# meffmadd/intro-tc-vae

Measured on AMD Instinct MI355X. Metric: images/sec (64x64x3, z=128, bs=64) intro-TC step, higher is better.
Workload: dtype f32 in/out/accumulate, conv products on split-fp16 MFMA (two scaled fp16 planes, 3 products, fp32-class); 1 GPU; c2: IntroTCSovler.train_step, conv arch, 64x64x3, z_dim=128, channels (64, 128, 256, 512), batch 64/GPU, Adam lr 2e-4, clip 100, N=10000; global_batch=64, parallelism=single, sync_bn=False

## Files before the change

### include/itcv_hip.h

```cpp
#ifndef ITCV_HIP_H
#define ITCV_HIP_H

#include <stddef.h>
#include <stdint.h>

#ifdef __cplusplus
extern "C" {
#endif

#define ITCV_ABI_VERSION 4

int itcv_abi_version(void);
const char* itcv_last_error(void);
int itcv_set_option(const char* name, int value);
int itcv_get_option(const char* name);

int itcv_profile_begin(void);
int itcv_profile_end(void);
int itcv_profile_get(int i, int* code, double* flop, float* ms);
int itcv_profile_clear(void);

size_t itcv_conv2d_packed_weight_elems(int Co, int Ci, int KS, int for_dgrad);
int itcv_conv2d_pack_weight(const float* w, float* wp, int Co, int Ci, int KS, int for_dgrad,
                            void* stream);
size_t itcv_conv2d_fwd_workspace(int B, int Ci, int H, int W, int Co, int KS);
int itcv_conv2d_fwd(const float* x, const float* wp, const float* bias, float* y, int B, int Ci,
                    int H, int W, int Co, int KS, int up2, void* ws, size_t ws_bytes, void* stream);
int itcv_conv2d_bf16s_supported(int Ci, int Co, int KS);
size_t itcv_conv2d_packed_weight_bytes_bf16s(int Co, int Ci, int KS, int for_dgrad, int ns);
int itcv_conv2d_pack_weight_bf16s(const float* w, void* wp, int Co, int Ci, int KS, int for_dgrad, int ns,
                                  void* stream);
size_t itcv_pack_desc_bytes(void);
int itcv_conv2d_pack_desc_bf16s(void* host_desc, const float* w, void* wp, int Co, int Ci, int KS, int for_dgrad,
                                int ns, int block0);
int itcv_conv2d_pack_weights_bf16s(const void* dev_table, int n, int total_blocks, int ns, void* stream);
size_t itcv_conv2d_fwd_bf16s_workspace(int B, int Ci, int H, int W, int Co, int KS);
int itcv_conv2d_fwd_bf16s(const float* x, const void* wp, const float* bias, float* y, int B, int Ci, int H,
                          int W, int Co, int KS, int up2, int ns, void* ws, size_t ws_bytes, void* stream);
#define ITCV_PLANES_F16X2 4
size_t itcv_planes_bytes(int B, int C, int HW, int ns);
int itcv_split_planes(const float* x, void* planes, int B, int C, int HW, int ns, void* stream);
int itcv_absmax(const float* x, size_t n, float* parts, void* stream);
int itcv_split_planes_scaled(const float* x, void* planes, int B, int C, int HW, int ns, const float* amax, void* stream);
size_t itcv_conv2d_fwd_bf16p_workspace(int B, int Ci, int H, int W, int Co, int KS, int ns);
int itcv_conv2d_fwd_bf16p(const void* xplanes, const void* wp, const float* bias, float* y, int B, int Ci, int H,
                          int W, int Co, int KS, int up2, int ns, void* ws, size_t ws_bytes, void* stream);
int itcv_conv2d_fwd_bf16p_stat_tiles(int B, int Ci, int H, int W, int Co, int KS, int ns);
int itcv_conv2d_fwd_bf16p_st(const void* xplanes, const void* wp, const float* bias, float* y, int B, int Ci, int H,
                             int W, int Co, int KS, int up2, int ns, float* tile_stats, void* ws, size_t ws_bytes,
                             void* stream);
int itcv_conv2d_wgrad_bf16p_supported(int B, int Ci, int H, int W, int Co, int KS);
size_t itcv_conv2d_wgrad_bf16p_workspace(int B, int Ci, int H, int W, int Co, int KS);
int itcv_conv2d_wgrad_bf16p(const void* xplanes, const void* dyplanes, float* dw, int B, int Ci, int H, int W,
                            int Co, int KS, int up2, int ns , int accumulate, void* ws, size_t ws_bytes,
                            void* stream);
int itcv_conv2d_wgrad_bf16p_slabs(int B, int Ci, int H, int W, int Co, int KS);
size_t itcv_wgrad_reduce_desc_bytes(void);
int itcv_wgrad_reduce_desc(void* host_desc, const float* const* slabs, const int* splits, int nsrc, float* dw, int Co,
                           int Ci, int accumulate, int block0);
int itcv_wgrad_reduce_many(const void* dev_table, int n, int total_blocks, void* stream);
int itcv_wgrad_reduce_max_descs(void);
size_t itcv_linear_workspace(int B, int K, int N);
int itcv_linear_fwd(const float* x, const float* w, const float* bias, float* y, int B, int K, int N, void* ws,
                    size_t ws_bytes, void* stream);
int itcv_linear_dgrad(const float* dy, const float* w, float* dx, int B, int K, int N, void* ws, size_t ws_bytes,
                      void* stream);
int itcv_linear_wgrad(const float* dy, const float* x, float* dw, int B, int K, int N, int accumulate, void* ws,
                      size_t ws_bytes, void* stream);
int itcv_conv2d_wgrad5_bf16p_supported(int Cs, int Cb, int H, int W);
size_t itcv_conv2d_wgrad5_bf16p_workspace(int B, int H);
int itcv_conv2d_wgrad5_bf16p(const float* small, const void* big_planes, float* dw, int B, int Cs, int H, int W,
                             int stem, int ns , const float* small_amax ,
                             int accumulate, void* ws, size_t ws_bytes, void* stream);
int itcv_conv2d_small_cout_supported(int Co, int KS);
int itcv_conv2d_small_cout_bf16p_supported(int C, int Co, int KS);
int itcv_conv2d_small_cout_fwd_bf16p(const void* xplanes, const float* w, const float* bias, float* y, int B, int C,
                                     int H, int W, int Co, int KS, int for_dgrad, int ns , void* stream);
int itcv_conv2d_small_cout_fwd(const float* x, const float* w, const float* bias, float* y, int B, int C,
                               int H, int W, int Co, int KS, int for_dgrad, void* stream);
int itcv_conv2d_small_cin_supported(int C, int KS);
int itcv_conv2d_small_cin_fwd(const float* x, const float* w, const float* bias, float* y, int B, int C, int H,
                              int W, int Co, int KS, int for_dgrad, void* stream);

int itcv_conv2d_small_cin_bf16x3_supported(int C, int Co, int KS, int W);
int itcv_conv2d_small_cin_fwd_bf16x3(const float* x, const float* w, const float* bias, float* y, int B, int C, int H,
                                     int W, int Co, int KS, int for_dgrad, int ns ,
                                     const float* x_amax , void* stream);
int itcv_conv2d_wgrad_bf16s_supported(int Ci, int H, int W, int Co, int KS);
int itcv_conv2d_wgrad_bf16s(const float* x, const float* dy, float* dw, int B, int Ci, int H, int W, int Co,
                            int KS, int ns, int accumulate, void* ws, size_t ws_bytes, void* stream);
size_t itcv_conv2d_wgrad_workspace(int B, int Ci, int H, int W, int Co, int KS);
int itcv_conv2d_wgrad(const float* x, const float* dy, float* dw, int B, int Ci, int H, int W,
                      int Co, int KS, int up2, int accumulate, void* ws, size_t ws_bytes, void* stream);
int itcv_conv2d_fwd_variant(int B, int Ci, int H, int W, int Co, int KS, int up2);
int itcv_conv2d_wgrad_variant(int B, int Ci, int H, int W, int Co, int KS, int up2);
size_t itcv_bias_grad_workspace(int B, int C, int HW);
int itcv_bias_grad(const float* dy, float* db, int B, int C, int HW, int accumulate, void* ws,
                   size_t ws_bytes, void* stream);

size_t itcv_bn_workspace(int B, int C, int HW);
int itcv_bn_moments(const float* x, double* sums, int B, int C, int HW, void* ws, size_t ws_bytes,
                    void* stream);
int itcv_bn_train_stats(const float* x, int B, int C, int HW, float eps, float momentum, float* running_mean,
                        float* running_var, int64_t* num_batches_tracked, float* mean, float* rstd, void* ws,
                        size_t ws_bytes, void* stream);
int itcv_bn_finalize(const double* sums, double count, float eps, float momentum, float* running_mean,
                     float* running_var, int64_t* num_batches_tracked, float* mean, float* rstd, int C,
                     void* stream);
int itcv_bn_finalize_uv(const double* sums, double count, float eps, float momentum, float* running_mean,
                        float* running_var, int64_t* num_batches_tracked, float* mean, float* rstd, float* unbiased_var,
                        int C, void* stream);
int itcv_bn_eval_stats(const float* running_mean, const float* running_var, float eps, float* mean,
                       float* rstd, int C, void* stream);
int itcv_bn_act_fwd(const float* x, const float* mean, const float* rstd, const float* gamma,
                    const float* beta, const float* skip, float* y, int B, int C, int H, int W,
                    float slope, int pool, void* planes, int ns, size_t plane_stride, void* stream);
int itcv_bn_act_planes_supported(int C, int H, int W, int pool);
int itcv_bn_act_bwd_reduce(const float* x, const float* dy, const float* mean, const float* rstd,
                           const float* gamma, const float* beta, const float* skip, double* dsums,
                           float* dgamma, float* dbeta, int accumulate, int B, int C, int H, int W,
                           float slope, int pool, int up2, void* ws, size_t ws_bytes, void* stream);
int itcv_bn_act_bwd_apply(const float* x, const float* dy, const float* mean, const float* rstd,
                          const float* gamma, const float* beta, const float* skip, const double* dsums,
                          const double* local_dsums, double count, float* dx, float* dskip,
                          float* dgamma, float* dbeta, int accumulate, int B, int C, int H, int W,
                          float slope, int pool, int up2, void* dx_planes, int ns, size_t plane_stride, void* stream);

int itcv_bn_train_fwd(const float* x, const float* gamma, const float* beta, const float* skip, float* y, void* planes,
                      int ns, int B, int C, int H, int W, float slope, int pool, float eps, float momentum,
                      float* running_mean, float* running_var, int64_t* num_batches_tracked, float* mean, float* rstd,
                      void* ws, size_t ws_bytes, size_t plane_stride, const float* tile_stats, int tiles, int tile_pitch,
                      int groups, void* stream);
int itcv_bn_train_fwd_uv(const float* x, const float* gamma, const float* beta, const float* skip, float* y, void* planes,
                         int ns, int B, int C, int H, int W, float slope, int pool, float eps, float momentum,
                         float* running_mean, float* running_var, int64_t* num_batches_tracked, float* mean, float* rstd,
                         float* unbiased_var, void* ws, size_t ws_bytes, size_t plane_stride, const float* tile_stats,
                         int tiles, int tile_pitch, int groups, void* stream);
size_t itcv_bn_replay_desc_bytes(void);
int itcv_bn_replay_desc(void* host_desc, float* running_mean, float* running_var, int64_t* num_batches_tracked,
                        const float* mean, const float* unbiased_var, int C, int groups, float momentum, int block0);
int itcv_bn_replay_many(const void* dev_table, int n, int total_blocks, void* stream);
int itcv_bn_replay_max_descs(void);
int itcv_bn_train_bwd(const float* x, const float* dy, const float* mean, const float* rstd, const float* gamma,
                      const float* beta, const float* skip, double* dsums, float* dx, float* dskip, void* dx_planes,
                      int ns, float* dgamma, float* dbeta, int accumulate, int B, int C, int H, int W, float slope,
                      int pool, int up2, void* ws, size_t ws_bytes, size_t plane_stride, int groups, void* stream);

#define ITCV_BN_PATH_ONE_BLOCK 0
#define ITCV_BN_PATH_SLICED_FOLD 1
#define ITCV_BN_PATH_SLICED_COMBINE 2
#define ITCV_BN_PATH_FALLBACK 3
#define ITCV_BN_PATH_PER_GROUP 4
#define ITCV_BN_PATH_TILE_STATS 5
int itcv_bn_plan_query(int bwd, int B, int C, int H, int W, int pool, int up2, int groups, int planes, int ns,
                       size_t ws_bytes, int tile_stats, int* path, int* splits);

int itcv_lrelu_fwd(const float* x, float* y, size_t n, float slope, void* stream);
int itcv_lrelu_bwd(const float* x, const float* dy, float* dx, size_t n, float slope, void* stream);
int itcv_sigmoid_fwd(const float* x, float* y, size_t n, void* stream);
int itcv_sigmoid_bwd(const float* y, const float* dy, float* dx, size_t n, void* stream);
int itcv_avgpool2_fwd(const float* x, float* y, int BC, int H, int W, void* stream);
int itcv_avgpool2_bwd(const float* dy, float* dx, int BC, int H, int W, void* stream);
int itcv_upsample2_fwd(const float* x, float* y, int BC, int H, int W, void* stream);
int itcv_upsample2_bwd(const float* dy, float* dx, int BC, int H, int W, void* stream);
int itcv_add(const float* a, const float* b, float* out, size_t n, void* stream);

int itcv_reparam_fwd(const float* mu, const float* logvar, const float* eps, float* z, size_t n,
                     void* stream);
int itcv_reparam_bwd(const float* dz, const float* logvar, const float* eps, float* dmu, float* dlogvar,
                     size_t n, void* stream);
int itcv_kl_rows_fwd(const float* logvar, const float* mu, float* kl, int B, int D, void* stream);
int itcv_kl_rows_bwd(const float* g, const float* logvar, const float* mu, float* dlogvar, float* dmu,
                     int B, int D, void* stream);

#define ITCV_TC_VAR_FROM_ROW 0x1
#define ITCV_TC_EPS_DENSITY 0x2
#define ITCV_TC_WEIGHTED 0x4
#define ITCV_TC_LIVE (ITCV_TC_VAR_FROM_ROW | ITCV_TC_EPS_DENSITY)
size_t itcv_tc_fwd_workspace(int Bl, int Bt, int D);
int itcv_tc_fwd(const float* z, const float* mu_all, const float* logvar, float* prodm, float* logqz,
                float* lse, float* sjoint, int Bl, int Bt, int row_offset, int D, int64_t dataset_size, int flags,
                void* ws, size_t ws_bytes, void* stream);
size_t itcv_tc_bwd_workspace(int Bl, int Bt);
int itcv_tc_bwd(const float* g, const float* z, const float* mu_all, const float* logvar,
                const float* logqz, const float* lse, const float* sjoint, float* dz, float* dmu_all,
                float* dlogvar, int Bl, int Bt, int row_offset, int D, int64_t dataset_size, int flags, void* ws,
                size_t ws_bytes, void* stream);
int itcv_tc_kl_fwd(const float* z, const float* mu_all, const float* logvar, float* out, float* rows, float* prodm,
                   float* logqz, float* lse, float* sjoint, int Bl, int Bt, int row_offset, int D, int64_t dataset_size,
                   float coef_tc, float coef_kl, int reduction, void* ws, size_t ws_bytes, void* stream);
int itcv_tc_kl_bwd(const float* g, const float* z, const float* mu_all, const float* logvar, const float* logqz,
                   const float* lse, const float* sjoint, float* dz, float* dmu_all, float* dlogvar, int Bl, int Bt,
                   int row_offset, int D, int64_t dataset_size, float coef_tc, float coef_kl, int reduction, void* ws,
                   size_t ws_bytes, void* stream);
size_t itcv_tc_full_fwd_workspace(int Bl, int Bt, int D);
int itcv_tc_full_fwd(const float* z, const float* mu_all, const float* logvar_all, int ld, float* out, float* rows,
                     float* comps, float* prodm, float* logqz, float* lse, float* sjoint, float* ivar, int Bl, int Bt,
                     int row_offset, int D, int64_t dataset_size, float alpha, float beta, float gamma, int reduction,
                     void* ws, size_t ws_bytes, void* stream);
size_t itcv_tc_full_bwd_workspace(int Bl, int Bt);
int itcv_tc_full_bwd(const float* g, const float* z, const float* mu_all, const float* logvar_all, int ld,
                     const float* logqz, const float* lse, const float* sjoint, const float* ivar, float* dz, float* dmu_all,
                     float* dlogvar_all, int Bl, int Bt, int row_offset, int D, int64_t dataset_size, float alpha,
                     float beta, float gamma, int reduction, void* ws, size_t ws_bytes, void* stream);
int itcv_kl_loss_fwd(const float* logvar, const float* mu, float* out, int B, int D, int reduction, float scale, void* stream);
int itcv_kl_loss_bwd(const float* g, const float* logvar, const float* mu, float* dlogvar, float* dmu, int B, int D,
                     int reduction, float scale, void* stream);
int itcv_diag_logdensity_rows(const float* z, const float* mu, const float* logvar, float* logq_cx,
                              float* logpz, int B, int D, void* stream);
int itcv_gauss_logdensity_fwd(const float* x, const float* mu, const float* logvar, float* out, const int64_t* dims,
                              const int64_t* sx, const int64_t* sm, const int64_t* sl, int eps_density, void* stream);
int itcv_gauss_logdensity_bwd(const float* g, const float* x, const float* mu, const float* logvar, float* dx,
                              float* dlogvar, const int64_t* dims, const int64_t* sx, const int64_t* sm,
                              const int64_t* sl, int eps_density, void* stream);
int itcv_sampling_fwd(const float* lp, float* prodm, float* logqz, float* lse, float* sjoint, int B, int D,
                      int64_t dataset_size, int weighted, void* stream);
int itcv_sampling_bwd(const float* g_prodm, const float* g_logqz, const float* lp, const float* lse,
                      const float* sjoint, const float* logqz, float* dlp, int B, int D, int64_t dataset_size,
                      int weighted, void* stream);
int itcv_on_off_diag(const float* x, float* diag, float* off, int m, int n, void* stream);

size_t itcv_disent_minmax_workspace(int N, int D);
int itcv_disent_minmax(const float* mu, size_t ld, int N, int D, float* mn, float* mx, int* flags, void* ws,
                       size_t ws_bytes, void* stream);
int itcv_disent_bins(const float* mu, size_t ld, int N, int D, const float* mn, const float* mx, int bins, int* out,
                     void* stream);
size_t itcv_disent_counts_elems(int D, int fsum, int bins);
int itcv_disent_hist(const float* mu, size_t ld, const int* v, int N, int D, int K, const int* fsize, int bins,
                     const float* mn, const float* mx, unsigned* counts, unsigned* vcount, int* flags, void* stream);
// ... 109 lines not shown
```

### intro-tc-vae_amd/csrc/conv_igemm.hip

```cpp
#include "conv_shared.h"

namespace itcv {



constexpr uint32_t kOobBase = 0x80000000u;

__device__ __forceinline__ float buf_load_s(__amdgpu_buffer_rsrc_t r, uint32_t voff, uint32_t soff) {
  return __builtin_bit_cast(float, __builtin_amdgcn_raw_buffer_load_b32(r, voff, __builtin_amdgcn_readfirstlane(soff), 0));
}

__host__ __device__ inline int tile_rows_for(int M) { return M <= 32 ? 32 : (M <= 64 ? 64 : 128); }

struct ConvArgs {
  const float* x;
  const float* wp;
  const float* bias;
  float* y;
  int B, Ci, H, W, Co;
  int Cip, Mp, N;
  int mt, nt;
  int ktiles, ktiles_per_split, cpt;
  uint32_t x_bytes;
  size_t slab_stride;
// ... 2305 lines not shown

size_t itcv_conv2d_fwd_bf16s_workspace(int B, int Ci, int H, int W, int Co, int KS) {
  if (B <= 0 || Ci <= 0 || H <= 0 || W <= 0 || Co <= 0) return 0;
  return plan_fwd(kFwdSplit, B, Ci, H, W, Co, KS).ws_need;
}

size_t itcv_conv2d_fwd_bf16p_workspace(int B, int Ci, int H, int W, int Co, int KS, int ns) {
  if (B <= 0 || Ci <= 0 || H <= 0 || W <= 0 || Co <= 0) return 0;
  return plan_fwd_planes(B, Ci, H, W, Co, KS, planes_of_fmt(ns), false).ws_need;
}

int itcv_conv2d_fwd_bf16s(const float* x, const void* wp, const float* bias, float* y, int B, int Ci, int H, int W,
                          int Co, int KS, int up2, int ns, void* ws, size_t ws_bytes, void* stream) {
  if (int e = check_dims("itcv_conv2d_fwd_bf16s", B, Ci, H, W, Co, KS)) return e;
  ITCV_REQUIRE(x && wp && y && (ns == 2 || ns == 3), "itcv_conv2d_fwd_bf16s");
  if (!itcv_conv2d_bf16s_supported(Ci, Co, KS))
    return fail("%s: shape not supported by the split-bf16 kernel (Ci %% 32, Co > 32, KS 1/3)", "itcv_conv2d_fwd_bf16s");
  if (up2) ITCV_REQUIRE(H % 2 == 0 && W % 2 == 0, "itcv_conv2d_fwd_bf16s(up2)");
  const FwdPlan p = plan_fwd(kFwdSplit, B, Ci, H, W, Co, KS);
  const size_t out_elems = (size_t)B * Co * H * W;
  if (int e = check_ws("itcv_conv2d_fwd_bf16s", ws, ws_bytes, p.ws_need)) return e;
  ConvArgsB a;
  a.x = x;
  a.wp = static_cast<const u32x4*>(wp);
  a.bias = p.splits > 1 ? nullptr : bias;
  a.y = p.splits > 1 ? static_cast<float*>(ws) : y;
  a.B = B, a.Ci = Ci, a.H = H, a.W = W, a.Co = Co;
  a.Mp = p.mt * p.bm;
  a.N = B * H * W;
  a.mt = p.mt, a.nt = p.nt, a.ktiles = p.ktiles, a.ktiles_per_split = p.kps, a.cpt = p.cip / 32;
  a.x_bytes = (uint32_t)((size_t)B * Ci * (up2 ? (H / 2) * (W / 2) : H * W) * sizeof(float));
  a.slab_stride = p.splits > 1 ? out_elems : 0;
#ifdef ITCV_DIAG
  a.ablate = diag_ablate();
#endif
  hipStream_t st = S(stream);
  {
    ProfScope prof(st, kProfFwdB, KS, p.bm, up2 ? 1 : 0, ns, 2.0 * B * H * W * (double)Co * Ci * KS * KS);
    launch_fwd_b(a, p, KS, up2, ns, st);
  }
  ITCV_CHECK_LAUNCH("itcv_conv2d_fwd_bf16s");
  return reduce_fwd_splits("itcv_conv2d_fwd_bf16s(reduce)", ws, bias, y, out_elems, p.splits, H * W, Co, st);
}

size_t itcv_planes_bytes(int B, int C, int HW, int ns) {
  if (B <= 0 || C <= 0 || HW <= 0 || (C & 7) || !fmt_ok(ns)) return 0;
  return (size_t)planes_of_fmt(ns) * B * (C / 8) * HW * 16 + (ns == ITCV_PLANES_F16X2 ? sizeof(ScaleRec) : 0);
}

int itcv_absmax(const float* x, size_t n, float* parts, void* stream) {
  ITCV_REQUIRE(x && parts && n > 0 && (reinterpret_cast<uintptr_t>(x) & 15) == 0, "itcv_absmax");
  hipLaunchKernelGGL(absmax_kernel, dim3(kAbsmaxParts), dim3(256), 0, S(stream), x, n, parts);
  ITCV_CHECK_LAUNCH("itcv_absmax");
  return 0;
}

int itcv_split_planes_scaled(const float* x, void* planes, int B, int C, int HW, int ns, const float* amax, void* stream) {
  ITCV_REQUIRE(x && planes && B > 0 && C > 0 && HW > 0 && (C & 7) == 0 && fmt_ok(ns), "itcv_split_planes");
  ITCV_REQUIRE(!amax || ns == ITCV_PLANES_F16X2, "itcv_split_planes(a scale only applies to fp16 planes)");
  const size_t total = (size_t)B * (C / 8) * HW;
  const int blocks = (int)(cdivz(total, 256) < 8192 ? cdivz(total, 256) : 8192);
  pick_fmt(ns, [&](auto nsc, auto f16) {
    hipLaunchKernelGGL((split_planes_kernel<nsc.value, f16.value>), dim3(blocks), dim3(256), 0, S(stream), x,
                       static_cast<u32x4*>(planes), B, C / 8, HW, amax);
  });
  ITCV_CHECK_LAUNCH("itcv_split_planes");
  return 0;
}
int itcv_split_planes(const float* x, void* planes, int B, int C, int HW, int ns, void* stream) {
  return itcv_split_planes_scaled(x, planes, B, C, HW, ns, nullptr, stream);
}

int itcv_conv2d_fwd_bf16p(const void* xplanes, const void* wp, const float* bias, float* y, int B, int Ci, int H,
                          int W, int Co, int KS, int up2, int ns, void* ws, size_t ws_bytes, void* stream) {
  return itcv_conv2d_fwd_bf16p_st(xplanes, wp, bias, y, B, Ci, H, W, Co, KS, up2, ns, nullptr, ws, ws_bytes, stream);
}

int itcv_conv2d_fwd_bf16p_stat_tiles(int B, int Ci, int H, int W, int Co, int KS, int ns) {
  if (B <= 0 || Ci <= 0 || H <= 0 || W <= 0 || Co <= 0 || !itcv_conv2d_bf16s_supported(Ci, Co, KS)) return 0;
  if (ns == ITCV_PLANES_F16X2) return 0;
  return plan_fwd_planes(B, Ci, H, W, Co, KS, ns, true).stat_tiles;
}

int itcv_conv2d_fwd_bf16p_st(const void* xplanes, const void* wp, const float* bias, float* y, int B, int Ci, int H,
                             int W, int Co, int KS, int up2, int fmt, float* tile_stats, void* ws, size_t ws_bytes,
                             void* stream) {
  if (int e = check_dims("itcv_conv2d_fwd_bf16p", B, Ci, H, W, Co, KS)) return e;
  ITCV_REQUIRE(xplanes && wp && y && fmt_ok(fmt), "itcv_conv2d_fwd_bf16p");
  const int f16 = fmt == ITCV_PLANES_F16X2, ns = planes_of_fmt(fmt);
  if (tile_stats && (f16 || !itcv_conv2d_fwd_bf16p_stat_tiles(B, Ci, H, W, Co, KS, ns)))
    return fail("%s: tile statistics are not available for this shape / format (see itcv_conv2d_fwd_bf16p_stat_tiles)",
                "itcv_conv2d_fwd_bf16p_st");
  const size_t in_plane = (size_t)B * (Ci / 8) * (up2 ? (H / 2) * (W / 2) : H * W);
  const u32x4* xp = static_cast<const u32x4*>(xplanes);
  const ScaleRec* xrec = f16 ? reinterpret_cast<const ScaleRec*>(xp + 2 * in_plane) : nullptr;
  if (!itcv_conv2d_bf16s_supported(Ci, Co, KS))
    return fail("%s: shape not supported by the split-bf16 kernel (Ci %% 32, Co > 32, KS 1/3)", "itcv_conv2d_fwd_bf16p");
  if (up2) ITCV_REQUIRE(H % 2 == 0 && W % 2 == 0, "itcv_conv2d_fwd_bf16p(up2)");
  const size_t out_elems = (size_t)B * Co * H * W;
  const FwdPlanP p = plan_fwd_planes(B, Ci, H, W, Co, KS, ns, tile_stats != nullptr);
  if (int e = check_ws("itcv_conv2d_fwd_bf16p", ws, ws_bytes, p.ws_need)) return e;
  const bool split = p.splits > 1;
  const double flop = 2.0 * B * H * W * (double)Co * Ci * KS * KS;
  hipStream_t st = S(stream);
  if (p.path != FwdPath::Planes128) {
    ConvArgsP2 a;
    a.xp = xp;
    a.wp = static_cast<const u32x4*>(wp);
    a.bias = split ? nullptr : bias;
    a.y = split ? static_cast<float*>(ws) : y;
    a.B = B, a.Ci = Ci, a.H = H, a.Co = Co;
    a.Mp = p.mt * p.bm;
    a.N = B * H * W;
    a.mt = p.mt, a.nt = p.nt, a.cpt = p.cpt, a.cpt_per_split = p.cps;
    a.SR = p.SR, a.NSEG = p.NSEG, a.NP = p.NP, a.NPC = p.NPC, a.PXB = p.PXB;
    a.h_shift = log2_exact(H);
    a.stats = tile_stats, a.stat_T = p.nt;
    a.xscale = xrec;
    a.slab_stride = split ? out_elems : 0;
    a.plane_stride = in_plane;
#ifdef ITCV_DIAG
    a.debug = (diag_ablate() & 64) ? 1 : 0;
#endif
    {
      ProfScope prof(st, p.path == FwdPath::Band ? kProfFwdBand : kProfFwdBandPersist, log2_exact(W), p.bm, up2 ? 1 : 0, fmt, flop);
      launch_fwd_band(a, p, W, up2, f16, st);
    }
    ITCV_CHECK_LAUNCH("itcv_conv2d_fwd_bf16p(band)");
  } else {
    ConvArgsP a;
    a.xp = xp;
    a.wp = static_cast<const u32x4*>(wp);
    a.bias = split ? nullptr : bias;
    a.y = split ? static_cast<float*>(ws) : y;
    a.B = B, a.Ci = Ci, a.H = H, a.W = W, a.Co = Co;
    a.Mp = p.mt * p.bm;
    a.N = B * H * W;
    a.mt = p.mt, a.nt = p.nt, a.ktiles = p.ktiles, a.ktiles_per_split = p.kps;
    a.slab_stride = split ? out_elems : 0;
    a.plane_stride = in_plane;
    a.xscale = xrec;
#ifdef ITCV_DIAG
    a.ablate = diag_ablate();
#endif
    {
      ProfScope prof(st, kProfFwdP, KS, p.bm, up2 ? 1 : 0, fmt, flop);
      launch_fwd_p(a, p, KS, up2, fmt, st);
    }
    ITCV_CHECK_LAUNCH("itcv_conv2d_fwd_bf16p");
  }
  return reduce_fwd_splits("itcv_conv2d_fwd_bf16p(reduce)", ws, bias, y, out_elems, p.splits, H * W, Co, st);
}

size_t itcv_conv2d_wgrad_workspace(int B, int Ci, int H, int W, int Co, int KS) {
  if (B <= 0 || Ci <= 0 || H <= 0 || W <= 0 || Co <= 0) return 0;
  size_t n = plan_wgrad(B, Ci, H, W, Co, KS).ws_need;
  if (wgrad_swapped(Ci, Co)) {
    const size_t m = plan_wgrad(B, Co, H, W, Ci, KS).ws_need;
    if (m > n) n = m;
  }
  return n;
}

int itcv_conv2d_wgrad(const float* x, const float* dy, float* dw, int B, int Ci, int H, int W, int Co, int KS,
                      int up2, int accumulate, void* ws, size_t ws_bytes, void* stream) {
  if (int e = check_dims("itcv_conv2d_wgrad", B, Ci, H, W, Co, KS)) return e;
  ITCV_REQUIRE(x && dy && dw, "itcv_conv2d_wgrad");
  if (up2) ITCV_REQUIRE(H % 2 == 0 && W % 2 == 0, "itcv_conv2d_wgrad(up2)");
  const bool swapped = !up2 && wgrad_swapped(Ci, Co);
  WgradArgs a;
  const WgPlan p = plan_wgrad_call(a, x, dy, ws, B, Ci, H, W, Co, KS, up2, swapped, 32);
  if (int e = check_ws("itcv_conv2d_wgrad", ws, ws_bytes, p.ws_need)) return e;
  hipStream_t st = S(stream);
  {
    ProfScope prof(st, kProfWgrad, KS, p.bm, up2 ? 1 : 0, 0, 2.0 * B * H * W * (double)Co * Ci * KS * KS);
    launch_wgrad(a, p, KS, up2, st);
  }
  ITCV_CHECK_LAUNCH("itcv_conv2d_wgrad");
  const size_t dw_elems = (size_t)Co * Ci * KS * KS;
  const int blocks = (int)(cdivz(dw_elems, 256) < 2048 ? cdivz(dw_elems, 256) : 2048);
  if (dw_elems <= 65536 && p.splits >= 32)
    hipLaunchKernelGGL(splitk_reduce_wgrad_small, dim3((int)cdivz(dw_elems, 16)), dim3(256), 0, st,
                       static_cast<const float*>(ws), dw, Co, Ci, KS * KS, p.cip, p.cb, a.Np, p.slab, p.splits,
                       accumulate, swapped ? 1 : 0);
  else
    hipLaunchKernelGGL(splitk_reduce_wgrad, dim3(blocks), dim3(256), 0, st, static_cast<const float*>(ws), dw, Co, Ci,
                       KS * KS, p.cip, p.cb, a.Np, p.slab, p.splits, accumulate, swapped ? 1 : 0);
  ITCV_CHECK_LAUNCH("itcv_conv2d_wgrad(reduce)");
  return 0;
}

int itcv_conv2d_wgrad_bf16s_supported(int Ci, int H, int W, int Co, int KS) {
  return (KS == 1 || KS == 3) && Ci % 32 == 0 && W % 8 == 0 && Co >= 33 && H > 0;
}

int itcv_conv2d_wgrad_bf16s(const float* x, const float* dy, float* dw, int B, int Ci, int H, int W, int Co, int KS,
                            int ns, int accumulate, void* ws, size_t ws_bytes, void* stream) {
  if (int e = check_dims("itcv_conv2d_wgrad_bf16s", B, Ci, H, W, Co, KS)) return e;
  ITCV_REQUIRE(x && dy && dw && (ns == 2 || ns == 3), "itcv_conv2d_wgrad_bf16s");
  if (!itcv_conv2d_wgrad_bf16s_supported(Ci, H, W, Co, KS))
    return fail("%s: shape not supported by the split-bf16 kernel (Ci %% 32, W %% 8, Co > 32, KS 1/3)",
                "itcv_conv2d_wgrad_bf16s");
  WgradArgs a;
  const WgPlan p = plan_wgrad_call(a, x, dy, ws, B, Ci, H, W, Co, KS, 0, false, 64);
  if (int e = check_ws("itcv_conv2d_wgrad_bf16s", ws, ws_bytes, p.ws_need)) return e;
  hipStream_t st = S(stream);
  {
    ProfScope prof(st, kProfWgradB, KS, p.bm, 0, ns, 2.0 * B * H * W * (double)Co * Ci * KS * KS);
    launch_wgrad_b(a, p, KS, ns, st);
  }
  ITCV_CHECK_LAUNCH("itcv_conv2d_wgrad_bf16s");
  const size_t dw_elems = (size_t)Co * Ci * KS * KS;
  const int blocks = (int)(cdivz(dw_elems, 256) < 2048 ? cdivz(dw_elems, 256) : 2048);
  hipLaunchKernelGGL(splitk_reduce_wgrad, dim3(blocks), dim3(256), 0, st, static_cast<const float*>(ws), dw, Co, Ci,
                     KS * KS, p.cip, p.cb, a.Np, p.slab, p.splits, accumulate, 0);
  ITCV_CHECK_LAUNCH("itcv_conv2d_wgrad_bf16s(reduce)");
  return 0;
}

int itcv_conv2d_wgrad_bf16p_supported(int B, int Ci, int H, int W, int Co, int KS) {
  if (KS != 3 || B <= 0 || Ci < 8 || Co < 8 || (Ci & 7) || (Co & 7)) return 0;
  if (log2_exact(W) < 2 || W > 256 || log2_exact(H) < 0) return 0;
  const long long px = (long long)B * H * W;
  if (px % 64) return 0;
  if (H * W < 64 && 64 % (H * W)) return 0;
  return 1;
}

size_t itcv_conv2d_wgrad_bf16p_workspace(int B, int Ci, int H, int W, int Co, int KS) {
  if (!itcv_conv2d_wgrad_bf16p_supported(B, Ci, H, W, Co, KS)) return 0;
  return plan_wgrad_p(B, Ci, H, W, Co).ws_need;
}

int itcv_conv2d_wgrad_bf16p(const void* xplanes, const void* dyplanes, float* dw, int B, int Ci, int H, int W, int Co,
// ... 231 lines not shown
```

### intro-tc-vae_amd/csrc/norm_act.hip

```cpp
#include <stdlib.h>

#include <type_traits>

#include "common.h"

namespace itcv {

constexpr int kRedThreads = 256;

__device__ __forceinline__ uint32_t fdiv(uint32_t a, uint32_t d, int sh) { return sh >= 0 ? (a >> sh) : (a / d); }

struct BnGrp {
  size_t xs;
  size_t os;
  size_t dys;
  size_t ps;
  int cs;
  int G;
};

struct BnFinal {
  double count;
  float eps, momentum;
  float* running_mean;
  float* running_var;
  int64_t* nbt;
  float* mean;
  float* rstd;
  float* uvar;
};

__device__ __forceinline__ float bn_blend(float r, float s, float momentum) {
  float a = (1.f - momentum) * r, b = momentum * s;
  asm volatile("" : "+v"(a), "+v"(b));
  return a + b;
}

__device__ __forceinline__ void bn_finalize(double s1, double s2, double count, float eps, float momentum,
                                            float* running_mean, float* running_var, int c, float& mean_c, float& rstd_c,
                                            float* uvar_c = nullptr) {
  const double m = s1 / count;
  double var = s2 / count - m * m;
  if (var < 0.0) var = 0.0;
  mean_c = (float)m;
  rstd_c = (float)(1.0 / sqrt(var + (double)eps));
  if (running_mean) running_mean[c] = bn_blend(running_mean[c], (float)m, momentum);
  if (running_var) {
    const double unbiased = count > 1.0 ? var * count / (count - 1.0) : var;
    running_var[c] = bn_blend(running_var[c], (float)unbiased, momentum);
    if (uvar_c) *uvar_c = (float)unbiased;
  }
}

template <bool FUSED>
__global__ __launch_bounds__(kRedThreads) void bn_moments_partial(const float* __restrict__ x,
                                                                  double* __restrict__ part, int B, int C, int HW,
                                                                  int splits, int hw_shift, BnFinal f, BnGrp grp) {
  __shared__ double scratch[kRedThreads / 64];
  const uint32_t c = blockIdx.x, s = blockIdx.y, hw_n = HW, total = (uint32_t)B * hw_n;
  const uint32_t chunk = ((total + splits - 1) / splits + 3) & ~3u;
  const uint32_t beg = s * chunk, end = min(beg + chunk, total);
  const int ngroups = (FUSED && grp.G > 1) ? grp.G : 1;
  if (!FUSED) {
    x += (size_t)blockIdx.z * grp.xs;
    part += (size_t)blockIdx.z * splits * 2 * C;
  }
 for (int gi = 0; gi < ngroups; ++gi, x += grp.xs, f.mean += grp.cs, f.rstd += grp.cs) {
  double s1 = 0.0, s2 = 0.0;
  if ((HW & 3) == 0) {
#pragma unroll 4
    for (uint32_t i = beg + threadIdx.x * 4; i < end; i += kRedThreads * 4) {
      const uint32_t b = fdiv(i, hw_n, hw_shift), hw = i - b * hw_n;
      const float4 v = *reinterpret_cast<const float4*>(x + ((size_t)b * C + c) * hw_n + hw);
      s1 += ((double)v.x + (double)v.y) + ((double)v.z + (double)v.w);
      s2 += ((double)v.x * v.x + (double)v.y * v.y) + ((double)v.z * v.z + (double)v.w * v.w);
    }
  } else {
    for (uint32_t i = beg + threadIdx.x; i < end; i += kRedThreads) {
      const uint32_t b = fdiv(i, hw_n, hw_shift), hw = i - b * hw_n;
      const float v = x[((size_t)b * C + c) * hw_n + hw];
      s1 += (double)v;
      s2 += (double)v * v;
    }
  }
  s1 = block_sum(s1, scratch);
  s2 = block_sum(s2, scratch);
  if (threadIdx.x == 0) {
    if (FUSED) {
      bn_finalize(s1, s2, f.count, f.eps, f.momentum, f.running_mean, f.running_var, c, f.mean[c], f.rstd[c],
                  f.uvar ? f.uvar + (size_t)gi * grp.cs + c : nullptr);
      if (c == 0 && f.nbt) f.nbt[0] += 1;
    } else {
      part[((size_t)s * 2 + 0) * C + c] = s1;
      part[((size_t)s * 2 + 1) * C + c] = s2;
    }
  }
 }
}

__global__ void combine_partials(const double* __restrict__ part, double* __restrict__ sums, int C2, int splits) {
  const int i = blockIdx.x * blockDim.x + threadIdx.x;
  if (i >= C2) return;
// ... 347 lines not shown
  if (threadIdx.x == 0) {
    part[((size_t)s * 2 + 0) * C + c] = s1;
    part[((size_t)s * 2 + 1) * C + c] = s2;
  }
}

template <int MODE>
__global__ void bn_bwd_apply_kernel(const float* __restrict__ x, const float* __restrict__ dy,
                                    const float* __restrict__ mean, const float* __restrict__ rstd,
                                    const float* __restrict__ gamma, const float* __restrict__ beta,
                                    const float* __restrict__ skip, const double* __restrict__ dsums, double count,
                                    float* __restrict__ dx, float* __restrict__ dskip, int C, int H, int W,
                                    size_t n, float slope) {
  const int HW = H * W;
  for (size_t i = (size_t)blockIdx.x * blockDim.x + threadIdx.x; i < n; i += (size_t)gridDim.x * blockDim.x) {
    const size_t bc = i / HW;
    const int hw = (int)(i - bc * HW), h = hw / W, w = hw - h * W;
    const int c = (int)(bc % C);
    const float mu = mean[c], rs = rstd[c], ga = gamma[c];
    const float xh = (x[i] - mu) * rs;
    float u = xh * ga + beta[c];
    if (skip) u += skip[i];
    float g = upstream<MODE>(dy, bc, h, w, H, W);
    if (!(u > 0.f)) g *= slope;
    const float m1 = (float)(dsums[c] / count), m2 = (float)(dsums[C + c] / count);
    dx[i] = ga * rs * (g - m1 - xh * m2);
    if (dskip) dskip[i] = g;
  }
}



template <int MODE>
__device__ __forceinline__ float4 upstream4(const float* __restrict__ dy, uint32_t bc, uint32_t h, uint32_t w,
                                            uint32_t H, uint32_t W) {
  if (MODE == 0) return *reinterpret_cast<const float4*>(dy + (size_t)bc * H * W + h * W + w);
  if (MODE == 1) {
    const float2 d = *reinterpret_cast<const float2*>(dy + (size_t)bc * (H / 2) * (W / 2) + (h >> 1) * (W / 2) + (w >> 1));
    return make_float4(0.25f * d.x, 0.25f * d.x, 0.25f * d.y, 0.25f * d.y);
  }
  const float* p = dy + (size_t)bc * (4 * H * W) + (size_t)(2 * h) * (2 * W) + 2 * w;
  const float4 a0 = *reinterpret_cast<const float4*>(p), a1 = *reinterpret_cast<const float4*>(p + 4);
  const float4 b0 = *reinterpret_cast<const float4*>(p + 2 * W), b1 = *reinterpret_cast<const float4*>(p + 2 * W + 4);
  return make_float4((a0.x + a0.y) + (b0.x + b0.y), (a0.z + a0.w) + (b0.z + b0.w), (a1.x + a1.y) + (b1.x + b1.y),
                     (a1.z + a1.w) + (b1.z + b1.w));
}

struct BnBwdFinal {
  double* dsums;
  float* dgamma;
  float* dbeta;
  int accumulate;
};

template <int MODE, bool FUSED, bool MX = false>
__global__ __launch_bounds__(kRedThreads) void bn_bwd_partial_v4(
    const float* __restrict__ x, const float* __restrict__ dy, const float* __restrict__ mean,
    const float* __restrict__ rstd, const float* __restrict__ gamma, const float* __restrict__ beta,
    const float* __restrict__ skip, double* __restrict__ part, int B, int C, int H, int W, float slope, int splits,
    int w_shift, int hw_shift, BnBwdFinal f, BnGrp grp, float* __restrict__ mx = nullptr, int nmx = 0) {
  __shared__ double scratch[kRedThreads / 64];
  __shared__ float mscratch[MX ? 2 * (kRedThreads / 64) : 1];
  const uint32_t gz = FUSED ? 0u : blockIdx.z;
  const uint32_t c = blockIdx.x, s = blockIdx.y, HW = H * W, total = (uint32_t)B * HW;
  const uint32_t chunk = ((total + splits - 1) / splits + 3) & ~3u;
  const uint32_t beg = s * chunk, end = min(beg + chunk, total);
  const float ga = gamma[c], be = beta[c];
  const int ngroups = (FUSED && grp.G > 1) ? grp.G : 1;
  if (!FUSED) {
    const size_t g = blockIdx.z;
    x += g * grp.xs, dy += g * grp.dys, mean += g * grp.cs, rstd += g * grp.cs, part += g * splits * 2 * C;
    if (skip) skip += g * grp.xs;
  }
  float acc_db = 0.f, acc_dg = 0.f;
  if (FUSED && threadIdx.x == 0 && f.accumulate) {
    if (f.dbeta) acc_db = f.dbeta[c];
    if (f.dgamma) acc_dg = f.dgamma[c];
  }
 for (int gi = 0; gi < ngroups; ++gi, x += grp.xs, dy += grp.dys, mean += grp.cs, rstd += grp.cs, f.dsums += 2 * grp.cs) {
  if (skip && gi) skip += grp.xs;
  const float mu = mean[c], rs = rstd[c];
  double s1 = 0.0, s2 = 0.0;
  float gmax = 0.f, xmax = 0.f;
  constexpr int U = 4;
  for (uint32_t i0 = beg + threadIdx.x * 4; i0 < end; i0 += kRedThreads * 4 * U) {
    float4 xv4[U], g4[U], k4[U];
    bool ok[U];
#pragma unroll
    for (int u = 0; u < U; ++u) {
      const uint32_t iu = i0 + (uint32_t)u * kRedThreads * 4;
      ok[u] = iu < end;
      const uint32_t i = ok[u] ? iu : i0;
      const uint32_t b = fdiv(i, HW, hw_shift), hw = i - b * HW;
      const uint32_t h = fdiv(hw, W, w_shift), w = hw - h * W;
      const uint32_t bc = b * C + c;
      xv4[u] = *reinterpret_cast<const float4*>(x + (size_t)bc * HW + hw);
      g4[u] = upstream4<MODE>(dy, bc, h, w, H, W);
    }
    if (skip) {
#pragma unroll
      for (int u = 0; u < U; ++u) {
        const uint32_t iu = i0 + (uint32_t)u * kRedThreads * 4, i = iu < end ? iu : i0;
        const uint32_t b = fdiv(i, HW, hw_shift), hw = i - b * HW;
        k4[u] = *reinterpret_cast<const float4*>(skip + (size_t)(b * C + c) * HW + hw);
      }
    } else {
#pragma unroll
      for (int u = 0; u < U; ++u) k4[u] = make_float4(0.f, 0.f, 0.f, 0.f);
    }
#pragma unroll
    for (int u = 0; u < U; ++u) {
      const float4 xv = xv4[u];
      float4 g = g4[u];
      const float xh0 = (xv.x - mu) * rs, xh1 = (xv.y - mu) * rs, xh2 = (xv.z - mu) * rs, xh3 = (xv.w - mu) * rs;
      float u0 = xh0 * ga + be, u1 = xh1 * ga + be, u2 = xh2 * ga + be, u3 = xh3 * ga + be;
      if (skip) u0 += k4[u].x, u1 += k4[u].y, u2 += k4[u].z, u3 += k4[u].w;
      if (!(u0 > 0.f)) g.x *= slope;
      if (!(u1 > 0.f)) g.y *= slope;
      if (!(u2 > 0.f)) g.z *= slope;
      if (!(u3 > 0.f)) g.w *= slope;
      const double a1 = ((double)g.x + (double)g.y) + ((double)g.z + (double)g.w);
      const double a2 = ((double)g.x * xh0 + (double)g.y * xh1) + ((double)g.z * xh2 + (double)g.w * xh3);
      s1 += ok[u] ? a1 : 0.0;
      s2 += ok[u] ? a2 : 0.0;
      if constexpr (MX) {
        const float gm = fmaxf(fmaxf(fabsf(g.x), fabsf(g.y)), fmaxf(fabsf(g.z), fabsf(g.w)));
        const float xm = fmaxf(fmaxf(fabsf(xh0), fabsf(xh1)), fmaxf(fabsf(xh2), fabsf(xh3)));
        gmax = fmaxf(gmax, ok[u] ? gm : 0.f);
        xmax = fmaxf(xmax, ok[u] ? xm : 0.f);
      }
    }
  }
  s1 = block_sum(s1, scratch);
  s2 = block_sum(s2, scratch);
  if constexpr (MX) {
    gmax = wave_max(gmax), xmax = wave_max(xmax);
    if ((threadIdx.x & 63) == 0) mscratch[threadIdx.x >> 6] = gmax, mscratch[kRedThreads / 64 + (threadIdx.x >> 6)] = xmax;
    __syncthreads();
    if (threadIdx.x == 0) {
      float gm = 0.f, xm = 0.f;
      for (int k = 0; k < kRedThreads / 64; ++k) gm = fmaxf(gm, mscratch[k]), xm = fmaxf(xm, mscratch[kRedThreads / 64 + k]);
      const size_t idx = ((size_t)(FUSED ? (uint32_t)gi : gz) * splits + s) * C + c;
      mx[idx] = fabsf(ga * rs) * gm, mx[(size_t)nmx + idx] = xm;
    }
    __syncthreads();
  }
  if (threadIdx.x == 0) {
    if (FUSED) {
      f.dsums[c] = s1;
      f.dsums[C + c] = s2;
      acc_db += (float)s1, acc_dg += (float)s2;
    } else {
      part[((size_t)s * 2 + 0) * C + c] = s1;
      part[((size_t)s * 2 + 1) * C + c] = s2;
    }
  }
 }
  if (FUSED && threadIdx.x == 0) {
    if (f.dbeta) f.dbeta[c] = acc_db;
    if (f.dgamma) f.dgamma[c] = acc_dg;
  }
}

template <int MODE>
__global__ void bn_bwd_apply_v4(const float* __restrict__ x, const float* __restrict__ dy,
                                const float* __restrict__ mean, const float* __restrict__ rstd,
                                const float* __restrict__ gamma, const float* __restrict__ beta,
                                const float* __restrict__ skip, const double* __restrict__ dsums, double count,
                                float* __restrict__ dx, float* __restrict__ dskip, int C, int H, int W, uint32_t n4,
                                float slope, int w_shift, int hw_shift, int c_mask) {
  const uint32_t HW = H * W;
  for (uint32_t j = blockIdx.x * blockDim.x + threadIdx.x; j < n4; j += gridDim.x * blockDim.x) {
    const uint32_t i = j * 4;
    const uint32_t bc = fdiv(i, HW, hw_shift), hw = i - bc * HW;
    const uint32_t h = fdiv(hw, W, w_shift), w = hw - h * W;
    const uint32_t c = c_mask >= 0 ? (bc & (uint32_t)c_mask) : (bc % (uint32_t)C);
    const float mu = mean[c], rs = rstd[c], ga = gamma[c], be = beta[c];
    const float m1 = (float)(dsums[c] / count), m2 = (float)(dsums[C + c] / count), gr = ga * rs;
    const float4 xv = *reinterpret_cast<const float4*>(x + i);
    float4 g = upstream4<MODE>(dy, bc, h, w, H, W);
    const float xh0 = (xv.x - mu) * rs, xh1 = (xv.y - mu) * rs, xh2 = (xv.z - mu) * rs, xh3 = (xv.w - mu) * rs;
    float u0 = xh0 * ga + be, u1 = xh1 * ga + be, u2 = xh2 * ga + be, u3 = xh3 * ga + be;
    if (skip) {
      const float4 k = *reinterpret_cast<const float4*>(skip + i);
      u0 += k.x, u1 += k.y, u2 += k.z, u3 += k.w;
    }
    if (!(u0 > 0.f)) g.x *= slope;
    if (!(u1 > 0.f)) g.y *= slope;
    if (!(u2 > 0.f)) g.z *= slope;
    if (!(u3 > 0.f)) g.w *= slope;
    *reinterpret_cast<float4*>(dx + i) = make_float4(gr * (g.x - m1 - xh0 * m2), gr * (g.y - m1 - xh1 * m2),
                                                     gr * (g.z - m1 - xh2 * m2), gr * (g.w - m1 - xh3 * m2));
    if (dskip) *reinterpret_cast<float4*>(dskip + i) = g;
  }
}

struct BnBwdSumsIn {
  const double* part;
  int splits;
  double* dsums_out;
  float* dgamma;
  float* dbeta;
  int accumulate;
};

template <int MODE, int NS, bool SUMS, bool F16 = false>
__global__ __launch_bounds__(256) void bn_bwd_apply_planes(
    const float* __restrict__ x, const float* __restrict__ dy, const float* __restrict__ mean,
    const float* __restrict__ rstd, const float* __restrict__ gamma, const float* __restrict__ beta,
    const float* __restrict__ skip, const double* __restrict__ dsums, double count, float* __restrict__ dx,
    float* __restrict__ dskip, u32x4* __restrict__ planes, int B, int C, int H, int W, float slope, int w_shift,
    BnBwdSumsIn sm, size_t plane_stride, BnGrp grp, const float* __restrict__ mx = nullptr, int nmx = 0) {
  float pscale = 1.f;
  if constexpr (F16) {
    __shared__ float s_uv[8];
    float u = 0.f, v = 0.f;
    const float4* mu4 = reinterpret_cast<const float4*>(mx);
    const float4* mv4 = reinterpret_cast<const float4*>(mx + nmx);
    const int n4 = nmx >> 2;
    for (int i = threadIdx.x; i < n4; i += 4 * 256) {
      float4 tu[4], tv[4];
#pragma unroll
      for (int k = 0; k < 4; ++k) {
        const int idx = i + k * 256;
        tu[k] = idx < n4 ? mu4[idx] : make_float4(0.f, 0.f, 0.f, 0.f);
        tv[k] = idx < n4 ? mv4[idx] : make_float4(0.f, 0.f, 0.f, 0.f);
      }
#pragma unroll
      for (int k = 0; k < 4; ++k) {
        u = fmaxf(fmaxf(u, fmaxf(tu[k].x, tu[k].y)), fmaxf(tu[k].z, tu[k].w));
        v = fmaxf(fmaxf(v, fmaxf(tv[k].x, tv[k].y)), fmaxf(tv[k].z, tv[k].w));
      }
    }
    u = wave_max(u), v = wave_max(v);
    if ((threadIdx.x & 63) == 0) s_uv[threadIdx.x >> 6] = u, s_uv[4 + (threadIdx.x >> 6)] = v;
    __syncthreads();
    u = fmaxf(fmaxf(s_uv[0], s_uv[1]), fmaxf(s_uv[2], s_uv[3]));
    v = fmaxf(fmaxf(s_uv[4], s_uv[5]), fmaxf(s_uv[6], s_uv[7]));
    pscale = scale_for_bound(u * (2.f + v));
    if (blockIdx.x == 0 && blockIdx.z == 0 && threadIdx.x == 0) {
      ScaleRec* rec = reinterpret_cast<ScaleRec*>(planes + (size_t)NS * plane_stride);
      rec->scale = pscale, rec->inv = 1.f / pscale, rec->pad[0] = rec->pad[1] = 0.f;
    }
  }
  const uint32_t zg = gridDim.z - 1 - blockIdx.z;
  {
    const size_t g = zg;
    x += g * grp.xs, dy += g * grp.dys, planes += g * grp.ps, mean += g * grp.cs, rstd += g * grp.cs;
    if (dsums) dsums += g * 2 * grp.cs;
    if (skip) skip += g * grp.xs;
    if (dx) dx += g * grp.xs;
    if (dskip) dskip += g * grp.xs;
  }
  __shared__ float s_m1[SUMS ? kStatCh : 1], s_m2[SUMS ? kStatCh : 1];
  __shared__ u32x4 strips[4][64 * 4];
  const uint32_t HW = H * W, C8 = C >> 3, per_plane = HW / 4, total = (uint32_t)B * C8 * per_plane;
  const uint32_t sweep = gridDim.x * blockDim.x, rbase = (gridDim.x - 1 - blockIdx.x) * blockDim.x;
  for (int it = (int)((total + sweep - 1) / sweep) - 1; it >= 0; --it) {
    const uint32_t base = (uint32_t)it * sweep + rbase;
    if (base >= total) continue;
    const uint32_t idx = base + threadIdx.x;
    const uint32_t g0 = base / per_plane;
    if (SUMS) {
      __syncthreads();
      const uint32_t last = min(base + blockDim.x, total) - 1, ng = last / per_plane - g0 + 1;
      if (threadIdx.x < ng * 8) {
        const uint32_t gz = zg, G = grp.G > 1 ? grp.G : 1;
        const uint32_t g = g0 + threadIdx.x / 8, c = (g % C8) * 8 + (threadIdx.x & 7);
        const double* part = sm.part + (size_t)gz * sm.splits * 2 * C;
        const double s1 = fold_strided(0.0, part + c, (size_t)2 * C, sm.splits);
        const double s2 = fold_strided(0.0, part + C + c, (size_t)2 * C, sm.splits);
        s_m1[threadIdx.x] = (float)(s1 / count), s_m2[threadIdx.x] = (float)(s2 / count);
        if (g < C8 && g * per_plane >= base) {
          sm.dsums_out[(size_t)gz * 2 * C + c] = s1, sm.dsums_out[(size_t)gz * 2 * C + C + c] = s2;
          if (gz == 0) {
            float db = (sm.accumulate && sm.dbeta) ? sm.dbeta[c] : 0.f, dg = (sm.accumulate && sm.dgamma) ? sm.dgamma[c] : 0.f;
            db += (float)s1, dg += (float)s2;
            for (uint32_t gg = 1; gg < G; ++gg) {
              const double* pg = sm.part + (size_t)gg * sm.splits * 2 * C;
              db += (float)fold_strided(0.0, pg + c, (size_t)2 * C, sm.splits);
              dg += (float)fold_strided(0.0, pg + C + c, (size_t)2 * C, sm.splits);
            }
            if (sm.dbeta) sm.dbeta[c] = db;
            if (sm.dgamma) sm.dgamma[c] = dg;
          }
        }
      }
      __syncthreads();
    }
    if (idx >= total) continue;
    const uint32_t bc8 = idx / per_plane, p4 = idx - bc8 * per_plane;
    const uint32_t b = bc8 / C8, c8 = bc8 - b * C8;
    const uint32_t hw = p4 * 4, h = fdiv(hw, W, w_shift), w = hw - h * W;
    float o[8][4];
#pragma unroll
    for (int j0 = 0; j0 < 8; j0 += 4) {
      float4 xv4[4], g4[4], k4[4];
      float pm[4][4];
      double ds4[4][2];
#pragma unroll
      for (int jj = 0; jj < 4; ++jj) {
        const uint32_t c = c8 * 8 + j0 + jj, bc = b * C + c;
        xv4[jj] = *reinterpret_cast<const float4*>(x + bc * HW + hw);
        g4[jj] = upstream4<MODE>(dy, bc, h, w, H, W);
        pm[jj][0] = mean[c], pm[jj][1] = rstd[c], pm[jj][2] = gamma[c], pm[jj][3] = beta[c];
        if (!SUMS) ds4[jj][0] = dsums[c], ds4[jj][1] = dsums[C + c];
      }
      if (skip) {
#pragma unroll
        for (int jj = 0; jj < 4; ++jj) k4[jj] = *reinterpret_cast<const float4*>(skip + (b * C + c8 * 8 + j0 + jj) * HW + hw);
      } else {
#pragma unroll
        for (int jj = 0; jj < 4; ++jj) k4[jj] = make_float4(0.f, 0.f, 0.f, 0.f);
      }
#pragma unroll
      for (int jj = 0; jj < 4; ++jj) {
        const int j = j0 + jj;
        const uint32_t c = c8 * 8 + j, bc = b * C + c;
        const uint32_t i = bc * HW + hw;
        const float mu = pm[jj][0], rs = pm[jj][1], ga = pm[jj][2], be = pm[jj][3];
        const float m1 = SUMS ? s_m1[(bc8 - g0) * 8 + j] : (float)(ds4[jj][0] / count);
        const float m2 = SUMS ? s_m2[(bc8 - g0) * 8 + j] : (float)(ds4[jj][1] / count), gr = ga * rs;
        const float4 xv = xv4[jj];
        float4 g = g4[jj];
        const float xh0 = (xv.x - mu) * rs, xh1 = (xv.y - mu) * rs, xh2 = (xv.z - mu) * rs, xh3 = (xv.w - mu) * rs;
        float u0 = xh0 * ga + be, u1 = xh1 * ga + be, u2 = xh2 * ga + be, u3 = xh3 * ga + be;
        if (skip) {
          const float4 k = k4[jj];
          u0 += k.x, u1 += k.y, u2 += k.z, u3 += k.w;
        }
        if (!(u0 > 0.f)) g.x *= slope;
        if (!(u1 > 0.f)) g.y *= slope;
        if (!(u2 > 0.f)) g.z *= slope;
        if (!(u3 > 0.f)) g.w *= slope;
        const float4 d = make_float4(gr * (g.x - m1 - xh0 * m2), gr * (g.y - m1 - xh1 * m2), gr * (g.z - m1 - xh2 * m2),
                                     gr * (g.w - m1 - xh3 * m2));
        if (dx) *reinterpret_cast<float4*>(dx + i) = d;
        if (dskip) *reinterpret_cast<float4*>(dskip + i) = g;
        o[j][0] = d.x, o[j][1] = d.y, o[j][2] = d.z, o[j][3] = d.w;
      }
    }
    u32x4 chk[4][NS];
#pragma unroll
    for (int px = 0; px < 4; ++px) {
      float v8[8];
#pragma unroll
      for (int j = 0; j < 8; ++j) v8[j] = o[j][px];
      split8<NS, F16>(v8, chk[px], pscale);
    }
    const uint32_t cidx0 = base + (threadIdx.x & ~63u);
    if (cidx0 + 64 <= total) {
      store_planes_wave<4, NS>(planes, plane_stride, per_plane, HW, cidx0, chk, strips[threadIdx.x >> 6]);
    } else {
#pragma unroll
      for (int px = 0; px < 4; ++px)
#pragma unroll
        for (int p = 0; p < NS; ++p) planes[(size_t)p * plane_stride + (size_t)bc8 * HW + hw + px] = chk[px][p];
    }
  }
}

// ... 373 lines not shown

int itcv_bn_train_fwd_uv(const float* x, const float* gamma, const float* beta, const float* skip, float* y, void* planes,
                         int ns, int B, int C, int H, int W, float slope, int pool, float eps, float momentum,
                         float* running_mean, float* running_var, int64_t* num_batches_tracked, float* mean, float* rstd,
                         float* unbiased_var, void* ws, size_t ws_bytes, size_t plane_stride, const float* tile_stats,
                         int tiles, int tile_pitch, int groups, void* stream) {
  ITCV_REQUIRE(x && gamma && beta && mean && rstd && (y || planes) && B > 0 && C > 0 && H > 0 && W > 0, "itcv_bn_train_fwd");
  const double px_out = (double)(groups > 1 ? groups : 1) * B * C * (pool ? H * W / 4 : H * W);
  ProfScope bn_prof(S(stream), kProfBnFwd, ilog2_exact(W) >= 0 ? ilog2_exact(W) : 0, C / 8, pool ? 1 : 0, planes ? ns : 0,
                    (double)(groups > 1 ? groups : 1) * B * C * H * W * 4.0 * (skip ? 2 : 1) + px_out * ((planes ? 4.0 : 0.0) + (y ? 4.0 : 0.0)));
  if (groups > 1) ITCV_REQUIRE(!planes || plane_stride, "itcv_bn_train_fwd(groups need the plane stride of the whole tensor)");
  const BnPlan p = bn_plan(false, B, C, H, W, pool, 0, groups, planes != nullptr, ns, plane_stride, ws ? ws_bytes : 0,
                           tile_stats != nullptr);
  if (p.path == BnPath::PerGroup && planes && ns == ITCV_PLANES_F16X2)
    return fail("%s: fp16 planes need the merged group path (no tile statistics, a workspace of itcv_bn_workspace * groups)",
                "itcv_bn_train_fwd");
  if (p.path == BnPath::PerGroup) {
    const BnGrp& s = p.grp;
    for (int g = 0; g < groups; ++g)
      if (int e = itcv_bn_train_fwd_uv(x + g * s.xs, gamma, beta, skip ? skip + g * s.xs : nullptr, y ? y + g * s.os : nullptr,
                                       planes ? static_cast<u32x4*>(planes) + g * s.ps : nullptr, ns, B, C, H, W, slope, pool,
                                       eps, momentum, running_mean, running_var, num_batches_tracked, mean + (size_t)g * C,
                                       rstd + (size_t)g * C, unbiased_var ? unbiased_var + (size_t)g * C : nullptr, ws,
                                       ws_bytes, plane_stride, tile_stats ? tile_stats + (size_t)g * tiles : nullptr, tiles,
                                       tile_pitch, 1, stream))
        return e;
    return 0;
  }
  const BnFinal f{(double)B * H * W, eps, momentum, running_mean, running_var, num_batches_tracked, mean, rstd, unbiased_var};
  if (p.path == BnPath::TileStats) {
    ITCV_REQUIRE(tiles > 0 && tile_pitch >= tiles, "itcv_bn_train_fwd(tile statistics)");
    hipLaunchKernelGGL(bn_tile_stats_finalize_kernel, dim3(C), dim3(256), 0, S(stream), tile_stats, tiles, tile_pitch, f.count,
                       eps, momentum, running_mean, running_var, num_batches_tracked, mean, rstd, unbiased_var, C);
    ITCV_CHECK_LAUNCH("itcv_bn_train_fwd(tile statistics)");
  } else if (int e = bn_stats_launch(p, x, B, C, H * W, f, ws, ws_bytes, S(stream), "itcv_bn_train_fwd(statistics)")) {
    return e;
  }
  const BnStatsIn fold = p.path == BnPath::SlicedFold
                             ? BnStatsIn{static_cast<const double*>(ws), p.splits, f.count, eps, momentum, running_mean,
                                         running_var, num_batches_tracked, mean, rstd, unbiased_var}
                             : BnStatsIn{};
  return bn_fwd_apply_launch(p, x, mean, rstd, gamma, beta, skip, y, planes, ns, B, C, H, W, slope, pool, fold, S(stream));
}

int itcv_bn_train_fwd(const float* x, const float* gamma, const float* beta, const float* skip, float* y, void* planes,
                      int ns, int B, int C, int H, int W, float slope, int pool, float eps, float momentum,
                      float* running_mean, float* running_var, int64_t* num_batches_tracked, float* mean, float* rstd,
                      void* ws, size_t ws_bytes, size_t plane_stride, const float* tile_stats, int tiles, int tile_pitch,
                      int groups, void* stream) {
  return itcv_bn_train_fwd_uv(x, gamma, beta, skip, y, planes, ns, B, C, H, W, slope, pool, eps, momentum, running_mean,
                              running_var, num_batches_tracked, mean, rstd, nullptr, ws, ws_bytes, plane_stride, tile_stats,
                              tiles, tile_pitch, groups, stream);
}

size_t itcv_bn_replay_desc_bytes(void) { return sizeof(BnReplayDesc); }
int itcv_bn_replay_max_descs(void) { return kBnReplayMaxDesc; }
int itcv_bn_replay_desc(void* host_desc, float* running_mean, float* running_var, int64_t* num_batches_tracked,
                        const float* mean, const float* unbiased_var, int C, int groups, float momentum, int block0) {
  if (!(host_desc && C > 0 && groups >= 1 && block0 >= 0 && momentum >= 0.f && momentum <= 1.f) ||
      (running_mean && !mean) || (running_var && !unbiased_var)) {
    fail("%s: bad argument (descriptor, C > 0, groups >= 1, block0 >= 0, momentum in [0, 1], the saved statistics of every "
         "running buffer given)", "itcv_bn_replay_desc");
    return -1;
  }
  if (!running_mean && !running_var && !num_batches_tracked) return 0;
  BnReplayDesc d;
  memset(&d, 0, sizeof(d));
  d.running_mean = running_mean, d.running_var = running_var, d.nbt = num_batches_tracked;
  d.mean = mean, d.uvar = unbiased_var;
  d.C = C, d.G = groups, d.momentum = momentum, d.block0 = block0;
  memcpy(host_desc, &d, sizeof(d));
  return cdiv(C, 256);
}
int itcv_bn_replay_many(const void* dev_table, int n, int total_blocks, void* stream) {
  ITCV_REQUIRE(dev_table && n > 0 && total_blocks > 0, "itcv_bn_replay_many");
  if (n > kBnReplayMaxDesc)
    return fail("%s: at most %d descriptors per table (itcv_bn_replay_max_descs)", "itcv_bn_replay_many", kBnReplayMaxDesc);
  hipLaunchKernelGGL(bn_replay_many, dim3(total_blocks), dim3(256), 0, S(stream),
                     static_cast<const BnReplayDesc*>(dev_table), n);
  ITCV_CHECK_LAUNCH("itcv_bn_replay_many");
  return 0;
}

int itcv_bn_train_bwd(const float* x, const float* dy, const float* mean, const float* rstd, const float* gamma,
                      const float* beta, const float* skip, double* dsums, float* dx, float* dskip, void* dx_planes,
                      int ns, float* dgamma, float* dbeta, int accumulate, int B, int C, int H, int W, float slope,
                      int pool, int up2, void* ws, size_t ws_bytes, size_t plane_stride, int groups, void* stream) {
  ITCV_REQUIRE(x && dy && mean && rstd && gamma && beta && dsums && (dx || dx_planes) && B > 0 && C > 0,
               "itcv_bn_train_bwd");
  ITCV_REQUIRE(!(pool && up2), "itcv_bn_train_bwd(pool and up2 are exclusive)");
  const double bn_el = (double)(groups > 1 ? groups : 1) * B * C * H * W;
  ProfScope bn_prof(S(stream), kProfBnBwd, ilog2_exact(W) >= 0 ? ilog2_exact(W) : 0, C / 8, pool ? 1 : (up2 ? 2 : 0), dx_planes ? ns : 0,
                    bn_el * 4.0 * (1.0 + (pool ? 0.25 : (up2 ? 4.0 : 1.0)) + (skip ? 1.0 : 0.0)) +
                        bn_el * ((dx_planes ? 4.0 : 0.0) + (dx ? 4.0 : 0.0) + (dskip ? 4.0 : 0.0)));
  if (groups > 1) ITCV_REQUIRE(!dx_planes || plane_stride, "itcv_bn_train_bwd(groups need the plane stride of the whole tensor)");
  const BnPlan p = bn_plan(true, B, C, H, W, pool, up2, groups, dx_planes != nullptr, ns, plane_stride, ws ? ws_bytes : 0,
                           false);
  const size_t ws_need = p.ws_need;
  if (p.f16 && groups > 1 && (p.path == BnPath::PerGroup || !(ws && ws_bytes >= ws_need)))
    return fail("%s: fp16 gradient planes need the merged group path (W %% 4 == 0, planes, a workspace of itcv_bn_workspace * groups)",
                "itcv_bn_train_bwd");
  if (p.path == BnPath::PerGroup) {
    const BnGrp& s = p.grp;
    for (int g = 0; g < groups; ++g)
      if (int e = itcv_bn_train_bwd(x + g * s.xs, dy + g * s.dys, mean + (size_t)g * C, rstd + (size_t)g * C, gamma, beta,
                                    skip ? skip + g * s.xs : nullptr, dsums + (size_t)g * 2 * C, dx ? dx + g * s.xs : nullptr,
                                    dskip ? dskip + g * s.xs : nullptr,
                                    dx_planes ? static_cast<u32x4*>(dx_planes) + g * s.ps : nullptr, ns, dgamma, dbeta,
                                    (accumulate || g > 0) ? 1 : 0, B, C, H, W, slope, pool, up2, ws, ws_bytes, plane_stride,
                                    1, stream))
        return e;
    return 0;
  }
  if (p.f16) ITCV_REQUIRE(ws && ws_bytes >= ws_need, "itcv_bn_train_bwd(workspace, fp16 planes)");
  if (int e = bn_bwd_reduce_launch(p, x, dy, mean, rstd, gamma, beta, skip, dsums, dgamma, dbeta, accumulate, B, C, H, W, slope,
                                   ws, ws_bytes, S(stream), "itcv_bn_train_bwd(sums)"))
    return e;
  const BnBwdSumsIn fold = p.path == BnPath::SlicedFold
                               ? BnBwdSumsIn{static_cast<const double*>(ws), p.splits, dsums, dgamma, dbeta, accumulate}
                               : BnBwdSumsIn{};
  const float* mx = p.f16 ? reinterpret_cast<const float*>(static_cast<const double*>(ws) + p.part_doubles) : nullptr;
  return bn_bwd_apply_launch(p, x, dy, mean, rstd, gamma, beta, skip, dsums, (double)B * H * W, dx, dskip, dx_planes, ns, B, C,
                             H, W, slope, fold, mx, S(stream));
}

static_assert((int)BnPath::OneBlock == ITCV_BN_PATH_ONE_BLOCK && (int)BnPath::SlicedFold == ITCV_BN_PATH_SLICED_FOLD &&
                  (int)BnPath::SlicedCombine == ITCV_BN_PATH_SLICED_COMBINE && (int)BnPath::Fallback == ITCV_BN_PATH_FALLBACK &&
                  (int)BnPath::PerGroup == ITCV_BN_PATH_PER_GROUP && (int)BnPath::TileStats == ITCV_BN_PATH_TILE_STATS,
              "ITCV_BN_PATH_* follow BnPath");

int itcv_bn_plan_query(int bwd, int B, int C, int H, int W, int pool, int up2, int groups, int planes, int ns,
                       size_t ws_bytes, int tile_stats, int* path, int* splits) {
  ITCV_REQUIRE(B > 0 && C > 0 && H > 0 && W > 0, "itcv_bn_plan_query");
  const BnPlan p = bn_plan(bwd != 0, B, C, H, W, pool, up2, groups, planes != 0, ns, 0, ws_bytes, tile_stats != 0);
  if (path) *path = (int)p.path;
  if (splits) *splits = p.splits;
  return 0;
}

#define ITCV_POINTWISE(NAME, KERNEL, N, ...)                                                        \
  do {                                                                                              \
    if ((N) == 0) return 0;                                                                         \
    hipLaunchKernelGGL(KERNEL, dim3(grid_for(N)), dim3(256), 0, S(stream), __VA_ARGS__);            \
    ITCV_CHECK_LAUNCH(NAME);                                                                        \
    return 0;                                                                                       \
  } while (0)

int itcv_lrelu_fwd(const float* x, float* y, size_t n, float slope, void* stream) {
  ITCV_REQUIRE(x && y, "itcv_lrelu_fwd");
  ITCV_POINTWISE("itcv_lrelu_fwd", lrelu_fwd_kernel, n, x, y, n, slope);
}
int itcv_lrelu_bwd(const float* x, const float* dy, float* dx, size_t n, float slope, void* stream) {
  ITCV_REQUIRE(x && dy && dx, "itcv_lrelu_bwd");
  ITCV_POINTWISE("itcv_lrelu_bwd", lrelu_bwd_kernel, n, x, dy, dx, n, slope);
}
int itcv_sigmoid_fwd(const float* x, float* y, size_t n, void* stream) {
  ITCV_REQUIRE(x && y, "itcv_sigmoid_fwd");
  ITCV_POINTWISE("itcv_sigmoid_fwd", sigmoid_fwd_kernel, n, x, y, n);
}
int itcv_sigmoid_bwd(const float* y, const float* dy, float* dx, size_t n, void* stream) {
  ITCV_REQUIRE(y && dy && dx, "itcv_sigmoid_bwd");
  ITCV_POINTWISE("itcv_sigmoid_bwd", sigmoid_bwd_kernel, n, y, dy, dx, n);
}
int itcv_add(const float* a, const float* b, float* out, size_t n, void* stream) {
  ITCV_REQUIRE(a && b && out, "itcv_add");
  ITCV_POINTWISE("itcv_add", add_kernel, n, a, b, out, n);
}
int itcv_avgpool2_fwd(const float* x, float* y, int BC, int H, int W, void* stream) {
  ITCV_REQUIRE(x && y && BC > 0 && H > 0 && W > 0 && H % 2 == 0 && W % 2 == 0, "itcv_avgpool2_fwd");
  const size_t n = (size_t)BC * (H / 2) * (W / 2);
  ITCV_POINTWISE("itcv_avgpool2_fwd", avgpool2_fwd_kernel, n, x, y, H, W, n);
}
int itcv_avgpool2_bwd(const float* dy, float* dx, int BC, int H, int W, void* stream) {
  ITCV_REQUIRE(dy && dx && BC > 0 && H > 0 && W > 0 && H % 2 == 0 && W % 2 == 0, "itcv_avgpool2_bwd");
  const size_t n = (size_t)BC * H * W;
  ITCV_POINTWISE("itcv_avgpool2_bwd", avgpool2_bwd_kernel, n, dy, dx, H, W, n);
}
int itcv_upsample2_fwd(const float* x, float* y, int BC, int H, int W, void* stream) {
  ITCV_REQUIRE(x && y && BC > 0 && H > 0 && W > 0, "itcv_upsample2_fwd");
  const size_t n = (size_t)BC * H * W * 4;
  ITCV_POINTWISE("itcv_upsample2_fwd", upsample2_fwd_kernel, n, x, y, H, W, n);
}
int itcv_upsample2_bwd(const float* dy, float* dx, int BC, int H, int W, void* stream) {
  ITCV_REQUIRE(dy && dx && BC > 0 && H > 0 && W > 0, "itcv_upsample2_bwd");
  const size_t n = (size_t)BC * H * W;
  ITCV_POINTWISE("itcv_upsample2_bwd", upsample2_bwd_kernel, n, dy, dx, H, W, n);
}

}
```

### intro-tc-vae_amd/hipvae/abi.py

```python
import ctypes
import os
import subprocess

import torch

_HERE = os.path.dirname(os.path.abspath(__file__))
PKG_ROOT = os.path.dirname(_HERE)
LIB_PATH = os.environ.get("ITCV_LIB") or os.path.join(PKG_ROOT, "lib", "libitcv_hip.so")
CSRC = os.path.join(PKG_ROOT, "csrc")
ABI_VERSION = 4

p, i32, i64, sz, f32, f64 = (ctypes.c_void_p, ctypes.c_int, ctypes.c_int64, ctypes.c_size_t,
                             ctypes.c_float, ctypes.c_double)

SIGNATURES = {
    "itcv_abi_version": (i32, []),
    "itcv_last_error": (ctypes.c_char_p, []),
    "itcv_set_option": (i32, [ctypes.c_char_p, i32]),
    "itcv_get_option": (i32, [ctypes.c_char_p]),
    "itcv_profile_begin": (i32, []),
    "itcv_profile_end": (i32, []),
    "itcv_profile_get": (i32, [i32, p, p, p]),
    "itcv_profile_clear": (i32, []),
    "itcv_conv2d_packed_weight_elems": (sz, [i32, i32, i32, i32]),
    "itcv_conv2d_pack_weight": (i32, [p, p, i32, i32, i32, i32, p]),
    "itcv_conv2d_fwd_workspace": (sz, [i32] * 6),
    "itcv_conv2d_fwd": (i32, [p, p, p, p, i32, i32, i32, i32, i32, i32, i32, p, sz, p]),
    "itcv_conv2d_bf16s_supported": (i32, [i32, i32, i32]),
    "itcv_conv2d_packed_weight_bytes_bf16s": (sz, [i32] * 5),
    "itcv_conv2d_pack_weight_bf16s": (i32, [p, p, i32, i32, i32, i32, i32, p]),
    "itcv_pack_desc_bytes": (sz, []),
    "itcv_conv2d_pack_desc_bf16s": (i32, [p, p, p, i32, i32, i32, i32, i32, i32]),
    "itcv_conv2d_pack_weights_bf16s": (i32, [p, i32, i32, i32, p]),
    "itcv_conv2d_fwd_bf16s_workspace": (sz, [i32] * 6),
    "itcv_conv2d_fwd_bf16s": (i32, [p, p, p, p] + [i32] * 8 + [p, sz, p]),
    "itcv_planes_bytes": (sz, [i32] * 4),
    "itcv_split_planes": (i32, [p, p, i32, i32, i32, i32, p]),
    "itcv_absmax": (i32, [p, sz, p, p]),
    "itcv_split_planes_scaled": (i32, [p, p, i32, i32, i32, i32, p, p]),
    "itcv_conv2d_fwd_bf16p_workspace": (sz, [i32] * 7),
    "itcv_conv2d_fwd_bf16p": (i32, [p, p, p, p] + [i32] * 8 + [p, sz, p]),
    "itcv_conv2d_fwd_bf16p_stat_tiles": (i32, [i32] * 7),
    "itcv_conv2d_fwd_bf16p_st": (i32, [p, p, p, p] + [i32] * 8 + [p, p, sz, p]),
    "itcv_conv2d_wgrad_bf16p_supported": (i32, [i32] * 6),
    "itcv_conv2d_wgrad_bf16p_workspace": (sz, [i32] * 6),
    "itcv_conv2d_wgrad_bf16p": (i32, [p, p, p] + [i32] * 9 + [p, sz, p]),
    "itcv_conv2d_wgrad_bf16p_slabs": (i32, [i32] * 6),
    "itcv_wgrad_reduce_desc_bytes": (sz, []),
    "itcv_wgrad_reduce_desc": (i32, [p, p, p, i32, p, i32, i32, i32, i32]),
    "itcv_wgrad_reduce_many": (i32, [p, i32, i32, p]),
    "itcv_wgrad_reduce_max_descs": (i32, []),
    "itcv_linear_workspace": (sz, [i32] * 3),
    "itcv_linear_fwd": (i32, [p, p, p, p, i32, i32, i32, p, sz, p]),
    "itcv_linear_dgrad": (i32, [p, p, p, i32, i32, i32, p, sz, p]),
    "itcv_linear_wgrad": (i32, [p, p, p, i32, i32, i32, i32, p, sz, p]),
    "itcv_conv2d_wgrad5_bf16p_supported": (i32, [i32] * 4),
    "itcv_conv2d_wgrad5_bf16p_workspace": (sz, [i32, i32]),
    "itcv_conv2d_wgrad5_bf16p": (i32, [p, p, p] + [i32] * 6 + [p, i32, p, sz, p]),
    "itcv_conv2d_small_cout_supported": (i32, [i32, i32]),
    "itcv_conv2d_small_cout_bf16p_supported": (i32, [i32, i32, i32]),
    "itcv_conv2d_small_cout_fwd_bf16p": (i32, [p, p, p, p] + [i32] * 8 + [p]),
    "itcv_conv2d_small_cout_fwd": (i32, [p, p, p, p] + [i32] * 7 + [p]),
    "itcv_conv2d_small_cin_supported": (i32, [i32, i32]),
    "itcv_conv2d_small_cin_fwd": (i32, [p, p, p, p] + [i32] * 7 + [p]),
    "itcv_conv2d_small_cin_bf16x3_supported": (i32, [i32, i32, i32, i32]),
    "itcv_conv2d_small_cin_fwd_bf16x3": (i32, [p, p, p, p] + [i32] * 8 + [p, p]),
    "itcv_conv2d_wgrad_bf16s_supported": (i32, [i32] * 5),
    "itcv_conv2d_wgrad_bf16s": (i32, [p, p, p] + [i32] * 8 + [p, sz, p]),
    "itcv_conv2d_wgrad_workspace": (sz, [i32] * 6),
    "itcv_conv2d_wgrad": (i32, [p, p, p, i32, i32, i32, i32, i32, i32, i32, i32, p, sz, p]),
    "itcv_conv2d_fwd_variant": (i32, [i32] * 7),
    "itcv_conv2d_wgrad_variant": (i32, [i32] * 7),
    "itcv_bias_grad_workspace": (sz, [i32, i32, i32]),
    "itcv_bias_grad": (i32, [p, p, i32, i32, i32, i32, p, sz, p]),
    "itcv_bn_workspace": (sz, [i32, i32, i32]),
    "itcv_bn_moments": (i32, [p, p, i32, i32, i32, p, sz, p]),
    "itcv_bn_train_stats": (i32, [p, i32, i32, i32, f32, f32, p, p, p, p, p, p, sz, p]),
    "itcv_bn_finalize": (i32, [p, f64, f32, f32, p, p, p, p, p, i32, p]),
    "itcv_bn_finalize_uv": (i32, [p, f64, f32, f32, p, p, p, p, p, p, i32, p]),
    "itcv_bn_eval_stats": (i32, [p, p, f32, p, p, i32, p]),
    "itcv_bn_act_planes_supported": (i32, [i32] * 4),
    "itcv_bn_act_fwd": (i32, [p, p, p, p, p, p, p, i32, i32, i32, i32, f32, i32, p, i32, sz, p]),
    "itcv_bn_act_bwd_reduce": (i32, [p, p, p, p, p, p, p, p, p, p, i32, i32, i32, i32, i32, f32, i32, i32, p, sz,
                                     p]),
    "itcv_bn_act_bwd_apply": (i32, [p, p, p, p, p, p, p, p, p, f64, p, p, p, p, i32, i32, i32, i32, i32, f32,
                                    i32, i32, p, i32, sz, p]),
    "itcv_bn_train_fwd": (i32, [p, p, p, p, p, p, i32, i32, i32, i32, i32, f32, i32, f32, f32, p, p, p, p, p, p, sz, sz, p, i32, i32,
                                i32, p]),
    "itcv_bn_train_fwd_uv": (i32, [p, p, p, p, p, p, i32, i32, i32, i32, i32, f32, i32, f32, f32, p, p, p, p, p, p, p, sz, sz, p, i32,
                                   i32, i32, p]),
    "itcv_bn_replay_desc_bytes": (sz, []),
    "itcv_bn_replay_desc": (i32, [p, p, p, p, p, p, i32, i32, f32, i32]),
    "itcv_bn_replay_many": (i32, [p, i32, i32, p]),
    "itcv_bn_replay_max_descs": (i32, []),
    "itcv_bn_train_bwd": (i32, [p, p, p, p, p, p, p, p, p, p, p, i32, p, p, i32, i32, i32, i32, i32, f32, i32, i32, p,
                                sz, sz, i32, p]),
    "itcv_bn_plan_query": (i32, [i32] * 10 + [sz, i32, p, p]),
    "itcv_lrelu_fwd": (i32, [p, p, sz, f32, p]),
    "itcv_lrelu_bwd": (i32, [p, p, p, sz, f32, p]),
    "itcv_sigmoid_fwd": (i32, [p, p, sz, p]),
    "itcv_sigmoid_bwd": (i32, [p, p, p, sz, p]),
    "itcv_avgpool2_fwd": (i32, [p, p, i32, i32, i32, p]),
    "itcv_avgpool2_bwd": (i32, [p, p, i32, i32, i32, p]),
    "itcv_upsample2_fwd": (i32, [p, p, i32, i32, i32, p]),
    "itcv_upsample2_bwd": (i32, [p, p, i32, i32, i32, p]),
    "itcv_add": (i32, [p, p, p, sz, p]),
    "itcv_reparam_fwd": (i32, [p, p, p, p, sz, p]),
    "itcv_reparam_bwd": (i32, [p, p, p, p, p, sz, p]),
    "itcv_kl_rows_fwd": (i32, [p, p, p, i32, i32, p]),
    "itcv_kl_rows_bwd": (i32, [p, p, p, p, p, i32, i32, p]),
    "itcv_tc_fwd_workspace": (sz, [i32, i32, i32]),
    "itcv_tc_fwd": (i32, [p, p, p, p, p, p, p, i32, i32, i32, i32, i64, i32, p, sz, p]),
    "itcv_tc_bwd_workspace": (sz, [i32, i32]),
    "itcv_tc_bwd": (i32, [p, p, p, p, p, p, p, p, p, p, i32, i32, i32, i32, i64, i32, p, sz, p]),
    "itcv_tc_kl_fwd": (i32, [p] * 9 + [i32, i32, i32, i32, i64, f32, f32, i32, p, sz, p]),
    "itcv_tc_kl_bwd": (i32, [p] * 10 + [i32, i32, i32, i32, i64, f32, f32, i32, p, sz, p]),
    "itcv_tc_full_fwd_workspace": (sz, [i32, i32, i32]),
    "itcv_tc_full_fwd": (i32, [p, p, p, i32] + [p] * 8 + [i32, i32, i32, i32, i64, f32, f32, f32, i32, p, sz, p]),
    "itcv_tc_full_bwd_workspace": (sz, [i32, i32]),
    "itcv_tc_full_bwd": (i32, [p, p, p, p, i32] + [p] * 7 + [i32, i32, i32, i32, i64, f32, f32, f32, i32, p, sz, p]),
    "itcv_kl_loss_fwd": (i32, [p, p, p, i32, i32, i32, f32, p]),
    "itcv_kl_loss_bwd": (i32, [p, p, p, p, p, i32, i32, i32, f32, p]),
    "itcv_diag_logdensity_rows": (i32, [p, p, p, p, p, i32, i32, p]),
    "itcv_gauss_logdensity_fwd": (i32, [p, p, p, p, p, p, p, p, i32, p]),
    "itcv_gauss_logdensity_bwd": (i32, [p, p, p, p, p, p, p, p, p, p, i32, p]),
    "itcv_sampling_fwd": (i32, [p, p, p, p, p, i32, i32, i64, i32, p]),
    "itcv_sampling_bwd": (i32, [p, p, p, p, p, p, p, i32, i32, i64, i32, p]),
    "itcv_on_off_diag": (i32, [p, p, p, i32, i32, p]),
    "itcv_disent_minmax_workspace": (sz, [i32, i32]),
    "itcv_disent_minmax": (i32, [p, sz, i32, i32, p, p, p, p, sz, p]),
    "itcv_disent_bins": (i32, [p, sz, i32, i32, p, p, i32, p, p]),
    "itcv_disent_counts_elems": (sz, [i32, i32, i32]),
    "itcv_disent_hist": (i32, [p, sz, p, i32, i32, i32, p, i32, p, p, p, p, p, p]),
    "itcv_disent_mi": (i32, [p, p, i32, i32, i32, p, i32, p, p, p]),
    "itcv_logreg_colstats_workspace": (sz, [i32, i32]),
    "itcv_logreg_colstats": (i32, [p, sz, i32, i32, p, p, p, p, sz, p]),
    "itcv_logreg_workspace": (sz, [i32] * 4),
    "itcv_logreg_valgrad": (i32, [p, sz, p, p, p, i32, i32, i32, p, p, p, f64, p, p, p, p, sz, p]),
    "itcv_logreg_proba": (i32, [p, sz, p, p, p, i32, i32, i32, p, p, p, p, p, p, p]),
    "itcv_logreg_auc": (i32, [p, p, i32, i32, p, p, p, p, p, p, p]),
    "itcv_zdiff_row": (i32, [p, p, sz, i32, i32, p, p]),
    "itcv_gbt_workspace": (sz, [i32] * 6),
    "itcv_gbt_cuts": (i32, [p, i32, i32, i32, p, p, p]),
    "itcv_gbt_bin": (i32, [p, sz, i32, i32, i32, p, p, p, p, p]),
    "itcv_gbt_grad": (i32, [p, p, i32, i32, p, p, p, p, p, p, p, p]),
    "itcv_gbt_hist": (i32, [p, i32, i32, i32, p, p, p, p, i32, i32, i32, p, sz, p]),
    "itcv_gbt_split": (i32, [p, p, i32, i32, p, i32, i32, i32, f64, f64, p, p, p, p, p, p]),
    "itcv_gbt_advance": (i32, [p, i32, i32, p, p, p, i32, p, p]),
    "itcv_gbt_margins": (i32, [p, i32, i32, p, p, p, p, p, i32, p, p]),
    "itcv_gbt_predict": (i32, [p, p, i32, i32, p, p, p, p, p, p]),
    "itcv_gbt_importance": (i32, [p, p, i32, i32, p, i32, p, p]),
    "itcv_gbt_round": (i32, [p, i32, i32, i32, p, p, i32, p, p, p, p, i32, p, i32, f64, f64] + [p] * 5 + [sz] + [p] * 6),
    "itcv_fvae_gvar": (i32, [p, sz, i32, i32, p, p, p]),
    "itcv_fvae_votes": (i32, [p, sz, i32, i32, i32, p, f64, p, i32, p, p, p]),
    "itcv_fvae_classify": (i32, [p, p, i32, i32, i32, i32, p, f64, p, p, p]),
    "itcv_sap_svc_lds_rows": (i32, []),
    "itcv_sap_svc_workspace": (sz, [i32] * 4),
    "itcv_sap_svc_fit": (i32, [p, sz, p, i32, i32, i32, p, f64, f64, i32, p, p, p, p, p, p, sz, p]),
    "itcv_sap_svc_score": (i32, [p, sz, p, i32, i32, i32, p, p, p, p, p, p, p]),
    "itcv_recon_workspace": (sz, [i32, sz]),
    "itcv_recon_rows_fwd": (i32, [p, p, p, i32, sz, i32, p, sz, p]),
    "itcv_recon_rows_bwd": (i32, [p, p, p, p, i32, sz, i32, p]),
    "itcv_recon_loss_fwd": (i32, [p, p, p, i32, sz, i32, i32, f32, p, sz, p]),
    "itcv_recon_loss_bwd": (i32, [p, p, p, p, i32, sz, i32, i32, f32, p]),
    "itcv_exp_elbo_fwd": (i32, [p, p, p, p, i32, f32, p]),
    "itcv_exp_elbo_bwd": (i32, [p, p, p, p, i32, p]),
    "itcv_lincomb_fwd": (i32, [p, p, i32, p, p]),
    "itcv_lincomb_bwd": (i32, [p, p, i32, p, p]),
    "itcv_sumsq_workspace": (sz, [sz]),
    "itcv_sumsq": (i32, [p, sz, p, p, sz, p]),
    "itcv_clip_coef": (i32, [p, i32, f64, p, p, p]),
    "itcv_scale_by_dev": (i32, [p, sz, p, p]),
    "itcv_adam_step": (i32, [p, p, p, p, sz, f32, f32, f32, f32, i32, p]),
    "itcv_adam_step_dev": (i32, [p, p, p, p, sz, f32, f32, f32, f32, p, p]),
    "itcv_adamx_step_dev": (i32, [p] * 6 + [sz] + [f64] * 5 + [i32, p, p]),
    "itcv_sgd_step_dev": (i32, [p] * 4 + [sz] + [f64] * 4 + [i32, p, p]),
    "itcv_adagrad_step_dev": (i32, [p] * 4 + [sz] + [f64] * 4 + [i32, p, p]),
    "itcv_rmsprop_step_dev": (i32, [p] * 6 + [sz] + [f64] * 5 + [i32, p, p]),
    "itcv_fill": (i32, [p, sz, f32, p]),
# ... 101 lines not shown
```

### intro-tc-vae_amd/hipvae/functional.py

```python
import contextlib
import weakref

import torch
import torch.distributed as dist
from torch.autograd import Function
from torch.autograd.function import once_differentiable

from . import abi
from .abi import call, lib, ptr, stream

F32 = torch.float32


def set_option(name, value):
    call("itcv_set_option", name.encode(), int(value))


def get_option(name):
    return lib.itcv_get_option(name.encode())


@contextlib.contextmanager
def option_scope(name, value):
    prev = get_option(name)
    set_option(name, value)
    try:
        yield
    finally:
        set_option(name, prev)


def _ws(nbytes, device):
    return torch.empty(max(int(nbytes), 16), dtype=torch.uint8, device=device)


def _f32c(t):
    if t.dtype != F32:
        raise abi.HipExtensionError(f"HIP path is fp32 only (got {t.dtype})")
    return t if t.is_contiguous() else t.contiguous()


_DIRECT = [False]


@contextlib.contextmanager
def direct_grad_accumulation():
    prev, _DIRECT[0] = _DIRECT[0], True
    try:
        yield
    finally:
        _DIRECT[0] = prev


def _grad_target(param):
    g = param.grad if _DIRECT[0] else None
    return g if (g is not None and g.is_contiguous() and g.dtype == F32) else None


_SHARED_PASS = [None]


class SharedPass:

    def __init__(self):
        self.param_grads = True
        self.input_grad = True
        self.records = []
        self._first = False
        self._pool = {}
        self._tables = {}

    @contextlib.contextmanager
    def record(self):
        prev, _SHARED_PASS[0] = _SHARED_PASS[0], self
        self.records, self._first = [], True
        self.param_grads = self.input_grad = True
        try:
            yield self
        finally:
            _SHARED_PASS[0] = prev

    def _claim_first(self):
        first, self._first = self._first, False
        return first

    def _stats(self, G, C, device):
        k = (len(self.records), G, C, str(device))
        buf = self._pool.get(k)
        if buf is None:
            buf = self._pool[k] = torch.empty((2, G, C), dtype=F32, device=device)
        return buf

    def replay(self):
        replay_bn_running(self.records, self._tables)


def _shared_ok(ctx, what):
    sp = ctx.shared
    return sp is None or getattr(sp, what)


def replay_bn_running(records, tables=None):
    import ctypes
    if tables is None:
        tables = {}
    recs = [r for r in records if r[0] is not None or r[1] is not None or r[2] is not None]
    if not recs:
        return
    key = tuple((0 if r[0] is None else r[0].data_ptr(), 0 if r[1] is None else r[1].data_ptr(),
                 0 if r[2] is None else r[2].data_ptr(), r[3].data_ptr(), r[4].data_ptr(), tuple(r[3].shape), r[5])
                for r in recs)
    tab = tables.get(key)
    if tab is None:
        if len(recs) > lib.itcv_bn_replay_max_descs():
            raise abi.HipExtensionError("replay_bn_running: more BatchNorm layers than one table holds")
        nb = lib.itcv_bn_replay_desc_bytes()
        host = (ctypes.c_uint8 * (nb * len(recs)))()
        blocks = 0
        for i, (rm, rv, nbt, mean, uvar, momentum) in enumerate(recs):
            G, C = mean.shape
            got = lib.itcv_bn_replay_desc(ctypes.byref(host, i * nb), ptr(rm), ptr(rv), ptr(nbt), ptr(mean), ptr(uvar), C, G,
                                          float(momentum), blocks)
            if got <= 0:
                raise abi.HipExtensionError("itcv_bn_replay_desc: " + abi.last_error())
            blocks += got
        tab = tables[key] = (torch.frombuffer(bytearray(host), dtype=torch.uint8).to(recs[0][3].device), len(recs), blocks,
                             recs)
    call("itcv_bn_replay_many", ptr(tab[0]), tab[1], tab[2], stream())




_WEIGHT_EPOCH = [0]
_PACK_CACHE = {}


_PARAM_EPOCH = {}


def bump_weight_epoch(params=None):
    if params is None:
        _WEIGHT_EPOCH[0] += 1
        return
    for p in params:
        _PARAM_EPOCH[id(p)] = _PARAM_EPOCH.get(id(p), 0) + 1


_NS = {"fp32": 0, "bf16x3": 2, "bf16x6": 3, "f16x3": 4}
F16X2 = 4
import os as _os

_CONV_MATH = [_os.environ.get("ITCV_CONV_MATH", "fp32")]
assert _CONV_MATH[0] in _NS, "ITCV_CONV_MATH must be one of fp32 / bf16x3 / bf16x6 / f16x3"


def _two(ns):
    return ns in (2, F16X2)


_SMALL_PLANES = [True]
_POISON = [False]
_PLANES = [True]


def set_conv_math(mode):
    assert mode in _NS, mode
    _CONV_MATH[0] = mode


def conv_math():
    return _CONV_MATH[0]


@contextlib.contextmanager
def conv_math_scope(mode):
    if mode is None:
        yield
        return
    assert mode in _NS, mode
    prev, _CONV_MATH[0] = _CONV_MATH[0], mode
    try:
        yield
# ... 21 lines not shown
    wp = ent[1].get((for_dgrad, ns))
    if wp is None:
        grp = _PACK_GROUPS.get(id(weight)) if ns and _PACK_BATCH[0] else None
        if grp is not None:
            wp = grp.pack(weight, w4, for_dgrad, ns)
        else:
            wp = ent[1][(for_dgrad, ns)] = pack_weight(w4, for_dgrad) if ns == 0 else pack_weight_bf16s(w4, for_dgrad, ns)
    return wp


_PACK_BATCH = [True]
_PACK_GROUPS = {}


class _PackGroup:

    def __init__(self):
        self.members = {}
        self.tables = {}

    def pack(self, weight, w4, for_dgrad, ns):
        k = (for_dgrad, ns)
        mem = self.members.setdefault(k, {})
        rec = mem.get(id(weight))
        if rec is None or rec[2] != w4.data_ptr() or rec[1] != tuple(w4.shape[:3]):
            wp = pack_weight_bf16s(w4, for_dgrad, ns)
            mem[id(weight)] = [weakref.ref(weight), tuple(w4.shape[:3]), w4.data_ptr(), wp]
            self.tables.pop(k, None)
            _pack_entry(weight, _pack_key(weight))[1][k] = wp
            return wp
        stale = [i for i, r in mem.items()
                 if r[0]() is None or r[0]().data_ptr() != r[2] or tuple(r[0]().shape[:3]) != r[1]]
        if stale:
            for i in stale:
                del mem[i]
            self.tables.pop(k, None)
        tab = self.tables.get(k)
        if tab is None:
            tab = self.tables[k] = self._build(mem, for_dgrad, ns, weight.device)
        call("itcv_conv2d_pack_weights_bf16s", ptr(tab[0]), tab[1], tab[2], ns, stream())
        for r in mem.values():
            m = r[0]()
            _pack_entry(m, _pack_key(m))[1][k] = r[3]
        return rec[3]

    @staticmethod
    def _build(mem, for_dgrad, ns, device):
        import ctypes

        nb = lib.itcv_pack_desc_bytes()
        host = (ctypes.c_uint8 * (nb * len(mem)))()
        blocks = 0
        for i, r in enumerate(mem.values()):
            co, ci, ks = r[1]
            got = lib.itcv_conv2d_pack_desc_bf16s(ctypes.byref(host, i * nb), r[2], ptr(r[3]), co, ci, ks, int(for_dgrad), ns,
                                                  blocks)
            if got <= 0:
                raise abi.HipExtensionError("itcv_conv2d_pack_desc_bf16s: " + abi.last_error())
            blocks += got
        dev_table = torch.frombuffer(bytearray(host), dtype=torch.uint8).to(device)
        return dev_table, len(mem), blocks


def register_pack_group(params):
    grp = _PackGroup()
    for p in params:
        if p.dim() == 4:
            _PACK_GROUPS[id(p)] = grp
            weakref.finalize(p, _PACK_GROUPS.pop, id(p), None)
    return grp


def pack_weight_bf16s(w4, for_dgrad, ns):
    co, ci, ks = w4.shape[0], w4.shape[1], w4.shape[2]
    nbytes = lib.itcv_conv2d_packed_weight_bytes_bf16s(co, ci, ks, int(for_dgrad), ns)
    wp = torch.empty(nbytes // 4, dtype=torch.int32, device=w4.device)
    call("itcv_conv2d_pack_weight_bf16s", ptr(w4), ptr(wp), co, ci, ks, int(for_dgrad), ns, stream())
    return wp


_SCIN_MFMA = [True]


def conv_apply(x, weight, w4, for_dgrad, bias, B, Ci, H, W, Co, KS, up2):
    if not up2 and lib.itcv_conv2d_small_cout_supported(Co, KS):
        y = torch.empty((B, Co, H, W), dtype=F32, device=x.device)

        call("itcv_conv2d_small_cout_fwd", ptr(x), ptr(w4), ptr(bias), ptr(y), B, Ci, H, W, Co, KS, int(for_dgrad),
             stream())
        return y
    if not up2 and lib.itcv_conv2d_small_cin_supported(Ci, KS):
        y = torch.empty((B, Co, H, W), dtype=F32, device=x.device)
        fmt = _NS[_CONV_MATH[0]]
        if _SCIN_MFMA[0] and _two(fmt) and lib.itcv_conv2d_small_cin_bf16x3_supported(Ci, Co, KS, W):
            amax = absmax_parts(x) if (fmt == F16X2 and for_dgrad) else None
            call("itcv_conv2d_small_cin_fwd_bf16x3", ptr(x), ptr(w4), ptr(bias), ptr(y), B, Ci, H, W, Co, KS,
                 int(for_dgrad), fmt, ptr(amax), stream())
            return y

        call("itcv_conv2d_small_cin_fwd", ptr(x), ptr(w4), ptr(bias), ptr(y), B, Ci, H, W, Co, KS, int(for_dgrad),
             stream())
        return y
    ns = _NS[_CONV_MATH[0]]
    if ns in (2, 3) and lib.itcv_conv2d_bf16s_supported(Ci, Co, KS):
        wp = packed_weight(weight, w4, for_dgrad, ns)
        y = torch.empty((B, Co, H, W), dtype=F32, device=x.device)
        nws = lib.itcv_conv2d_fwd_bf16s_workspace(B, Ci, H, W, Co, KS)
        ws = _ws(nws, x.device) if nws else None

        call("itcv_conv2d_fwd_bf16s", ptr(x), ptr(wp), ptr(bias), ptr(y), B, Ci, H, W, Co, KS, int(up2), ns, ptr(ws), nws,
             stream())
        return y
    return conv_fwd_raw(x, packed_weight(weight, w4, for_dgrad), bias, B, Ci, H, W, Co, KS, up2)


def absmax_parts(x):
    parts = torch.empty(256, dtype=F32, device=x.device)
    call("itcv_absmax", ptr(x), x.numel(), ptr(parts), stream())
    return parts


def split_planes(x, ns, gradient=False):
    B, C, H, W = x.shape
    nbytes = lib.itcv_planes_bytes(B, C, H * W, ns)
    if not nbytes:
        raise abi.HipExtensionError(f"split_planes: unsupported shape {tuple(x.shape)} / ns={ns}")
    xp = torch.empty(nbytes // 4, dtype=torch.int32, device=x.device)
    if ns == F16X2 and gradient:
        call("itcv_split_planes_scaled", ptr(x), ptr(xp), B, C, H * W, ns, ptr(absmax_parts(x)), stream())
    else:
        call("itcv_split_planes", ptr(x), ptr(xp), B, C, H * W, ns, stream())
    return xp


_FUSE_STATS = [False]


def conv_apply_planes(xp, weight, w4, for_dgrad, bias, B, Ci, H, W, Co, KS, up2, ns, want_stats=False):
    if not up2 and _two(ns) and lib.itcv_conv2d_small_cout_bf16p_supported(Ci, Co, KS):
        y = torch.empty((B, Co, H, W), dtype=F32, device=xp.device)
        call("itcv_conv2d_small_cout_fwd_bf16p", ptr(xp), ptr(w4), ptr(bias), ptr(y), B, Ci, H, W, Co, KS, int(for_dgrad),
             ns, stream())
        return y
    wp = packed_weight(weight, w4, for_dgrad, ns)
    y = torch.empty((B, Co, H, W), dtype=F32, device=xp.device)
    nws = lib.itcv_conv2d_fwd_bf16p_workspace(B, Ci, H, W, Co, KS, ns)
    ws = _ws(nws, xp.device) if nws else None
    T = lib.itcv_conv2d_fwd_bf16p_stat_tiles(B, Ci, H, W, Co, KS, ns) if (want_stats and _FUSE_STATS[0]) else 0
    stats = torch.empty((2, Co, T), dtype=F32, device=xp.device) if T else None
    call("itcv_conv2d_fwd_bf16p_st", ptr(xp), ptr(wp), ptr(bias), ptr(y), B, Ci, H, W, Co, KS, int(up2), ns, ptr(stats),
         ptr(ws), nws, stream())
    if stats is not None:
        y._itcv_tile_stats = (stats, T, 256, y._version, y.data_ptr())
    return y


def _tile_stats_of(x, B, G, HW):
    tag = getattr(x, "_itcv_tile_stats", None)
    if tag is None or tag[3] != x._version or tag[4] != x.data_ptr():
        return None
    stats, T, px = tag[0], tag[1], tag[2]
    if T * px != B * HW or (B // G * HW) % px:
        return None
    return stats, T // G, T


_DEFER = {"on": False, "pending": [], "pool": {}, "tables": {}}


@contextlib.contextmanager
def deferred_wgrad_reduces():
    prev, _DEFER["on"] = _DEFER["on"], True
    try:
        yield
    finally:
        _DEFER["on"] = prev
        if not prev:
            flush_wgrad_reduces()


def flush_wgrad_reduces():
    pend = _DEFER["pending"]
    if not pend:
        return
    import ctypes
    groups = {}
    for ws, dw, co, ci, slabs in pend:
        groups.setdefault(dw.data_ptr(), [dw, co, ci, []])[3].append((ws, slabs))
    key = tuple((k, tuple((w.data_ptr(), n) for w, n in g[3])) for k, g in groups.items())
    tab = _DEFER["tables"].get(key)
    if tab is None:
        nb = lib.itcv_wgrad_reduce_desc_bytes()
        descs, blocks = [], 0
        for dw, co, ci, srcs in groups.values():
            for c0 in range(0, len(srcs), 4):
                part = srcs[c0:c0 + 4]
                descs.append((dw, co, ci, part, 1))
        host = (ctypes.c_uint8 * (nb * len(descs)))()
        for i, (dw, co, ci, part, acc) in enumerate(descs):
            sl = (ctypes.c_void_p * len(part))(*[w.data_ptr() for w, _ in part])
            sp = (ctypes.c_int * len(part))(*[n for _, n in part])
            got = lib.itcv_wgrad_reduce_desc(ctypes.byref(host, i * nb), sl, sp, len(part), dw.data_ptr(), co, ci, acc, blocks)
            if got <= 0:
                raise abi.HipExtensionError("itcv_wgrad_reduce_desc: " + abi.last_error())
            blocks += got
        if len(descs) != len(groups):
            raise abi.HipExtensionError("deferred weight-gradient reduce: more than four passes over one weight")
        if len(_DEFER["tables"]) > 64:
            _DEFER["tables"].clear()
        tab = _DEFER["tables"][key] = (torch.frombuffer(bytearray(host), dtype=torch.uint8).to(pend[0][1].device), len(descs), blocks)
    call("itcv_wgrad_reduce_many", ptr(tab[0]), tab[1], tab[2], stream())
    pend.clear()


def _defer_slab_buffer(nbytes, device):
    k = (len(_DEFER["pending"]), int(nbytes), str(device))
    buf = _DEFER["pool"].get(k)
    if buf is None:
        buf = _DEFER["pool"][k] = torch.empty(max(int(nbytes), 16), dtype=torch.uint8, device=device)
    return buf

# ... 144 lines not shown
        ns = _NS[_CONV_MATH[0]]
    return ns


def conv_input_mode(conv, B, H, W, up2=False):
    ns = conv_input_planes_ns(conv, up2)
    if not ns:
        return 0, True
    ks = conv.kernel_size[0]
    wg_ok = (_wgrad_planes_ok(B, conv.in_channels, H, W, conv.out_channels, ks)
             or _wgrad5_mode(conv.in_channels, H, W, conv.out_channels, ks, up2) == "predict")
    return ns, not (_two(ns) and wg_ok)


def conv_grad_mode(conv, B, H, W, needs_input_grad=True):
    ns = conv_grad_planes_ns(conv, needs_input_grad)
    if not ns:
        return 0, True
    ks = conv.kernel_size[0]
    dgrad_ok = (not needs_input_grad) or _planes_ns(conv.out_channels, conv.in_channels, ks, False) == ns
    wgrad_ok = _two(ns) and _wgrad_planes_ok(B, conv.in_channels, H, W, conv.out_channels, ks)
    return ns, not (dgrad_ok and wgrad_ok and conv.bias is None)


def _planes_ns(Ci, Co, KS, up2):
    ns = _NS[_CONV_MATH[0]]
    if not ns or not _PLANES[0]:
        return 0
    if not up2 and _two(ns) and _SMALL_PLANES[0] and lib.itcv_conv2d_small_cout_bf16p_supported(Ci, Co, KS):
        return ns
    if not up2 and (lib.itcv_conv2d_small_cout_supported(Co, KS) or lib.itcv_conv2d_small_cin_supported(Ci, KS)):
        return 0
    return ns if lib.itcv_conv2d_bf16s_supported(Ci, Co, KS) else 0


def _wgrad5_mode(Ci, H, W, Co, KS, up2):
    if up2 or KS != 5 or not _two(_NS[_CONV_MATH[0]]) or not (_PLANES[0] and _SMALL_PLANES[0]):
        return None
    if Ci <= 3 and lib.itcv_conv2d_wgrad5_bf16p_supported(Ci, Co, H, W):
        return "stem"
    if Co <= 3 and lib.itcv_conv2d_wgrad5_bf16p_supported(Co, Ci, H, W):
        return "predict"
    return None


def conv_wgrad5_planes(small, big_planes, B, Cs, H, W, stem, out=None, accumulate=False, ns=2):
    dw = out if out is not None else torch.empty((64, Cs, 5, 5) if stem else (Cs, 64, 5, 5), dtype=F32, device=small.device)
    nws = lib.itcv_conv2d_wgrad5_bf16p_workspace(B, H)
    ws = _ws(nws, small.device)

    amax = absmax_parts(small) if (ns == F16X2 and not stem) else None
    call("itcv_conv2d_wgrad5_bf16p", ptr(small), ptr(big_planes), ptr(dw), B, Cs, H, W, int(stem), int(ns), ptr(amax),
         int(accumulate), ptr(ws), nws, stream())
    return dw


def _wgrad_planes_ok(B, Ci, H, W, Co, KS):
    return bool(_two(_NS[_CONV_MATH[0]]) and _PLANES[0] and lib.itcv_conv2d_wgrad_bf16p_supported(B, Ci, H, W, Co, KS))


class Conv2dFn(Function):

    @staticmethod
    def forward(ctx, x, weight, bias, up2):
        x, weight = _f32c(x), _f32c(weight)
        B, Ci, Hs, Ws = x.shape
        Co, KS = weight.shape[0], weight.shape[2]
        H, W = (Hs * 2, Ws * 2) if up2 else (Hs, Ws)
        b = None if bias is None else _f32c(bias)
        ns = _planes_ns(Ci, Co, KS, up2)
        xp = None
        if ns:
            xp = planes_of(x, ns)
            y = conv_apply_planes(xp, weight, weight, 0, b, B, Ci, H, W, Co, KS, up2, ns, want_stats=True)
        else:
            y = conv_apply(_require_fp32(x, "Conv2dFn.forward"), weight, weight, 0, b, B, Ci, H, W, Co, KS, up2)
        wg_planes = _wgrad_planes_ok(B, Ci, H, W, Co, KS)
        keep_xp = xp if (_two(ns) and (wg_planes or _wgrad5_mode(Ci, H, W, Co, KS, up2) == "predict")) else None
        ctx.save_for_backward(None if keep_xp is not None else _require_fp32(x, "Conv2dFn.forward (saved input)"),
                              weight, bias, keep_xp)
        ctx.cfg = (B, Ci, H, W, Co, KS, up2, bias is not None, (Hs, Ws))
        ctx.shared = _SHARED_PASS[0]
        ctx.shared_first = ctx.shared is not None and ctx.shared._claim_first()
        return y

    @staticmethod
    @once_differentiable
    def backward(ctx, dy):
        x, weight, bias, xp = ctx.saved_tensors
        B, Ci, H, W, Co, KS, up2, has_bias, (Hs, Ws) = ctx.cfg
        dy = _f32c(dy)
        dx = dw = db = None
        need_x = ctx.needs_input_grad[0] and not (ctx.shared_first and not ctx.shared.input_grad)
        need_w = ctx.needs_input_grad[1] and _shared_ok(ctx, "param_grads")
        need_b = ctx.needs_input_grad[2] and _shared_ok(ctx, "param_grads")
        ns_d = _planes_ns(Co, Ci, KS, False) if need_x else 0
        wg_planes = need_w and _wgrad_planes_ok(B, Ci, H, W, Co, KS)
        dyp = None
        fmt2 = F16X2 if _NS[_CONV_MATH[0]] == F16X2 else 2
        if ns_d or wg_planes:
            dyp = planes_of(dy, ns_d if ns_d else fmt2, gradient=True)
        if need_x:
            if ns_d:
                dx = conv_apply_planes(dyp, weight, weight, 1, None, B, Co, H, W, Ci, KS, False, ns_d)
            else:
                dx = conv_apply(_require_fp32(dy, "Conv2dFn.backward"), weight, weight, 1, None, B, Co, H, W, Ci, KS, False)
            if up2:
                lo = torch.empty((B, Ci, H // 2, W // 2), dtype=F32, device=dy.device)
                call("itcv_upsample2_bwd", ptr(dx), ptr(lo), B * Ci, H // 2, W // 2, stream())
                dx = lo
        wg5 = _wgrad5_mode(Ci, H, W, Co, KS, up2) if need_w else None
        if wg5 == "predict" and xp is None and x is None:
            wg5 = None
        if wg5 is not None:
            tgt = _grad_target(weight)
            if wg5 == "stem":
                small, big = _require_fp32(x, "Conv2dFn.backward (5x5 weight gradient)"), (dyp if dyp is not None else planes_of(dy, fmt2, gradient=True))
            else:
                small, big = _require_fp32(dy, "Conv2dFn.backward (5x5 weight gradient)"), (xp if xp is not None else split_planes(x, fmt2))
            cs = Ci if wg5 == "stem" else Co
            if tgt is not None:
                conv_wgrad5_planes(small, big, B, cs, H, W, wg5 == "stem", out=tgt, accumulate=True, ns=fmt2)
            else:
                dw = conv_wgrad5_planes(small, big, B, cs, H, W, wg5 == "stem", ns=fmt2)
        elif need_w:
            tgt = _grad_target(weight)
            if wg_planes and (ns_d in (0, fmt2)):
                if xp is None:
                    xp = split_planes(x, fmt2)
                if tgt is not None:
                    conv_wgrad_planes(xp, dyp, B, Ci, H, W, Co, KS, up2, out=tgt, accumulate=True, ns=fmt2)
                else:
                    dw = conv_wgrad_planes(xp, dyp, B, Ci, H, W, Co, KS, up2, ns=fmt2)
            else:
                if x is None:
                    raise abi.HipExtensionError("Conv2dFn.backward: conv math mode changed between forward and backward")
                _require_fp32(dy, "Conv2dFn.backward (weight gradient)")
                if tgt is not None:
                    conv_wgrad_raw(x, dy, B, Ci, H, W, Co, KS, up2, out=tgt, accumulate=True)
                else:
                    dw = conv_wgrad_raw(x, dy, B, Ci, H, W, Co, KS, up2)
        if has_bias and need_b:
            db = bias_grad_raw(_require_fp32(dy, "Conv2dFn.backward (bias gradient)"), B, Co, H * W, _grad_target(bias))
        return dx, dw, db, None


class LinearFn(Function):

    @staticmethod
    def forward(ctx, x, weight, bias):
        x, weight = _f32c(x), _f32c(weight)
        B, K = x.shape
        N = weight.shape[0]
        y = torch.empty((B, N), dtype=F32, device=x.device)
        nws = lib.itcv_linear_workspace(B, K, N)
        ws = _ws(nws, x.device) if nws else None
        call("itcv_linear_fwd", ptr(x), ptr(weight), ptr(None if bias is None else _f32c(bias)), ptr(y), B, K, N, ptr(ws),
             nws, stream())
        ctx.save_for_backward(x, weight, bias)
        ctx.cfg = (B, K, N, bias is not None)
        ctx.shared = _SHARED_PASS[0]
        ctx.shared_first = ctx.shared is not None and ctx.shared._claim_first()
        return y

    @staticmethod
    @once_differentiable
    def backward(ctx, dy):
        x, weight, bias = ctx.saved_tensors
        B, K, N, has_bias = ctx.cfg
        dy = _f32c(dy)
        dx = dw = db = None
        nws = lib.itcv_linear_workspace(B, K, N)
        need_p = _shared_ok(ctx, "param_grads")
        if ctx.needs_input_grad[0] and not (ctx.shared_first and not ctx.shared.input_grad):
            dx = torch.empty((B, K), dtype=F32, device=dy.device)
            ws = _ws(nws, dy.device) if nws else None
            call("itcv_linear_dgrad", ptr(dy), ptr(weight), ptr(dx), B, K, N, ptr(ws), nws, stream())
        if ctx.needs_input_grad[1] and need_p:
            tgt = _grad_target(weight)
            dw = None if tgt is not None else torch.empty((N, K), dtype=F32, device=dy.device)
            ws = _ws(nws, dy.device) if nws else None
            call("itcv_linear_wgrad", ptr(dy), ptr(x), ptr(tgt if tgt is not None else dw), B, K, N,
                 int(tgt is not None), ptr(ws), nws, stream())
        if has_bias and ctx.needs_input_grad[2] and need_p:
            db = bias_grad_raw(dy, B, N, 1, _grad_target(bias))
        return dx, dw, db


def _world(group):
    return dist.get_world_size(group) if (group is not None and dist.is_initialized()) else 1


class BnActFn(Function):

    @staticmethod
    def forward(ctx, x, gamma, beta, skip, running_mean, running_var, nbt, eps, momentum, slope, pool, training,
                group, out_planes=0, grad_planes=0, out_fp32=True, grad_fp32=True, bn_groups=1):
        x, gamma, beta = _f32c(x), _f32c(gamma), _f32c(beta)
        skip = None if skip is None else _f32c(skip)
        B, C, H, W = x.shape
        G = int(bn_groups) if training else 1
        if G < 1 or B % G:
            raise abi.HipExtensionError(f"BatchNorm groups: batch {B} is not {G} equal passes")
        Bg = B // G
        dev = x.device
        shared = _SHARED_PASS[0]
        uvar = None
        if shared is not None and training:
            mean, uvar = shared._stats(G, C, dev)
        else:
            mean = torch.empty((G, C), dtype=F32, device=dev)
        rstd = torch.empty((G, C), dtype=F32, device=dev)
        world = _world(group) if training else 1
        oshape = (B, C, H // 2, W // 2) if pool else (B, C, H, W)
        y = torch.empty(oshape, dtype=F32, device=dev)
        yp, pstride = None, 0
        if F16X2 in (out_planes, grad_planes) and not (training and world == 1):
            out_planes = 0 if out_planes == F16X2 else out_planes
            grad_planes = 0 if grad_planes == F16X2 else grad_planes
            out_fp32 = grad_fp32 = True
        if out_planes and lib.itcv_bn_act_planes_supported(C, H, W, int(pool)):
            yp = torch.empty(lib.itcv_planes_bytes(B, C, oshape[2] * oshape[3], out_planes) // 4, dtype=torch.int32,
                             device=dev)
            pstride = B * (C // 8) * oshape[2] * oshape[3]
        write_y = out_fp32 or yp is None or _POISON[0]
        nws = lib.itcv_bn_workspace(Bg, C, H * W) * G
        ts = _tile_stats_of(x, B, G, H * W) if (training and world == 1) else None
        if training and world == 1:
            ws = _ws(nws, dev)
            head = (ptr(x), ptr(gamma), ptr(beta), ptr(skip), ptr(y) if write_y else None, ptr(yp), int(out_planes), Bg, C, H,
                    W, float(slope), int(pool), float(eps), float(momentum), ptr(running_mean), ptr(running_var), ptr(nbt),
                    ptr(mean), ptr(rstd))
            tail = (ptr(ws), nws, pstride, None if ts is None else ts[0].data_ptr(), ts[1] if ts else 0, ts[2] if ts else 0,
                    G, stream())
            if uvar is None:
                call("itcv_bn_train_fwd", *head, *tail)
            else:
                call("itcv_bn_train_fwd_uv", *head, ptr(uvar), *tail)
        for g in (range(G) if not (training and world == 1) else ()):
            r = slice(g * Bg, (g + 1) * Bg)
            xg, yg = x[r], (y[r] if write_y else None)
            sg = None if skip is None else skip[r]
            ypg = None if yp is None else yp[g * Bg * (C // 8) * oshape[2] * oshape[3] * 4:]
            if training:
                ws = _ws(nws, dev)
                sums = torch.empty((2 * C,), dtype=torch.float64, device=dev)
                call("itcv_bn_moments", ptr(xg), ptr(sums), Bg, C, H * W, ptr(ws), nws, stream())
                dist.all_reduce(sums, group=group)
                call("itcv_bn_finalize_uv", ptr(sums), float(Bg * H * W * world), float(eps), float(momentum),
                     ptr(running_mean), ptr(running_var), ptr(nbt), ptr(mean[g]), ptr(rstd[g]),
                     None if uvar is None else ptr(uvar[g]), C, stream())
            else:
                call("itcv_bn_eval_stats", ptr(running_mean), ptr(running_var), float(eps), ptr(mean[g]), ptr(rstd[g]), C,
                     stream())
            call("itcv_bn_act_fwd", ptr(xg), ptr(mean[g]), ptr(rstd[g]), ptr(gamma), ptr(beta), ptr(sg), ptr(yg), Bg, C, H, W,
                 float(slope), int(pool), ptr(ypg), int(out_planes), pstride, stream())
        if yp is not None:
            if _POISON[0] and not out_fp32:
                y.fill_(float("nan"))
            _tag_planes(y, yp, out_planes, bool(out_fp32))
        if uvar is not None:
            shared.records.append((running_mean, running_var, nbt, mean, uvar, float(momentum)))
        ctx.shared = shared
        ctx.save_for_backward(x, gamma, beta, mean, rstd, skip)
        ctx.params = (gamma, beta)
        if not lib.itcv_bn_act_planes_supported(C, H, W, 0):
            grad_planes = 0
        ctx.cfg = (B, C, H, W, float(slope), int(pool), bool(training), group, world, int(grad_planes),
                   bool(grad_fp32) or not grad_planes, G)
        ctx.mark_non_differentiable(*[t for t in (running_mean, running_var, nbt) if t is not None])
        return y

    @staticmethod
    @once_differentiable
    def backward(ctx, dy):
        x, gamma, beta, mean, rstd, skip = ctx.saved_tensors
        B, C, H, W, slope, pool, training, group, world, grad_planes, grad_fp32, G = ctx.cfg
        if not training:
            raise abi.HipExtensionError("BatchNorm backward in eval mode is not part of the training hot path")
        dy = _f32c(dy)
        dev = x.device
        Bg = B // G
        nws = lib.itcv_bn_workspace(Bg, C, H * W) * G
        need_g = ctx.needs_input_grad[1] and _shared_ok(ctx, "param_grads")
        need_b = ctx.needs_input_grad[2] and _shared_ok(ctx, "param_grads")
        tg = _grad_target(gamma) if need_g else None
        tb = _grad_target(beta) if need_b else None
        direct = tg is not None and tb is not None
        dgamma = dbeta = None
        if direct:
            pg, pb = tg, tb
        else:
            dgamma = torch.empty_like(gamma) if need_g else None
            dbeta = torch.empty_like(beta) if need_b else None
            pg, pb = dgamma, dbeta
        dx = torch.empty_like(x)
        dskip = torch.empty_like(x) if (skip is not None and ctx.needs_input_grad[3]) else None
        dxp, pstride = None, 0
        if grad_planes:
            dxp = torch.empty(lib.itcv_planes_bytes(B, C, H * W, grad_planes) // 4, dtype=torch.int32, device=dev)
            pstride = B * (C // 8) * H * W
        write_dx = grad_fp32 or dxp is None or _POISON[0]
        if world == 1:
            ws = _ws(nws, dev)
            local = torch.empty((G, 2 * C), dtype=torch.float64, device=dev)
            call("itcv_bn_train_bwd", ptr(x), ptr(dy), ptr(mean), ptr(rstd), ptr(gamma), ptr(beta), ptr(skip), ptr(local),
                 ptr(dx) if write_dx else None, ptr(dskip), ptr(dxp), grad_planes, ptr(pg), ptr(pb), 1 if direct else 0, Bg,
                 C, H, W, slope, pool, 0, ptr(ws), nws, pstride, G, stream())
        for g in (range(G) if world != 1 else ()):
            r = slice(g * Bg, (g + 1) * Bg)
            acc = 1 if (direct or g > 0) else 0
            xg, dyg = x[r], dy[r]
            sg = None if skip is None else skip[r]
            dxg = dx[r] if write_dx else None
            dsg = None if dskip is None else dskip[r]
            dxpg = None if dxp is None else dxp[g * Bg * (C // 8) * H * W * 4:]
            ws = _ws(nws, dev)
            local = torch.empty((2 * C,), dtype=torch.float64, device=dev)
            call("itcv_bn_act_bwd_reduce", ptr(xg), ptr(dyg), ptr(mean[g]), ptr(rstd[g]), ptr(gamma), ptr(beta), ptr(sg),
                 ptr(local), ptr(pg), ptr(pb), acc, Bg, C, H, W, slope, pool, 0, ptr(ws), nws, stream())
            total = local.clone()
            dist.all_reduce(total, group=group)
            call("itcv_bn_act_bwd_apply", ptr(xg), ptr(dyg), ptr(mean[g]), ptr(rstd[g]), ptr(gamma), ptr(beta), ptr(sg),
                 ptr(total), None, float(Bg * H * W * world), ptr(dxg), ptr(dsg), None, None, 0, Bg, C, H, W, slope,
                 pool, 0, ptr(dxpg), grad_planes, pstride, stream())
        if dxp is not None:
            if _POISON[0] and not grad_fp32:
                dx.fill_(float("nan"))
            _tag_planes(dx, dxp, grad_planes, bool(grad_fp32))
        return (dx, dgamma, dbeta, dskip) + (None,) * 14


class LeakyReluFn(Function):
    @staticmethod
    def forward(ctx, x, slope):
        x = _f32c(x)
        y = torch.empty_like(x)
        call("itcv_lrelu_fwd", ptr(x), ptr(y), x.numel(), float(slope), stream())
        ctx.save_for_backward(x)
        ctx.slope = float(slope)
        return y

    @staticmethod
    @once_differentiable
    def backward(ctx, dy):
        (x,) = ctx.saved_tensors
        dy = _f32c(dy)
        dx = torch.empty_like(x)
        call("itcv_lrelu_bwd", ptr(x), ptr(dy), ptr(dx), x.numel(), ctx.slope, stream())
        return dx, None


class SigmoidFn(Function):
    @staticmethod
    def forward(ctx, x):
        x = _f32c(x)
        y = torch.empty_like(x)
        call("itcv_sigmoid_fwd", ptr(x), ptr(y), x.numel(), stream())
        ctx.save_for_backward(y)
        return y

    @staticmethod
    @once_differentiable
    def backward(ctx, dy):
        (y,) = ctx.saved_tensors
        dy = _f32c(dy)
        dx = torch.empty_like(y)
        call("itcv_sigmoid_bwd", ptr(y), ptr(dy), ptr(dx), y.numel(), stream())
        return dx


class AvgPool2Fn(Function):
    @staticmethod
    def forward(ctx, x):
        x = _f32c(x)
        B, C, H, W = x.shape
        y = torch.empty((B, C, H // 2, W // 2), dtype=F32, device=x.device)
        call("itcv_avgpool2_fwd", ptr(x), ptr(y), B * C, H, W, stream())
        ctx.shape = (B, C, H, W)
        return y

    @staticmethod
    @once_differentiable
    def backward(ctx, dy):
        B, C, H, W = ctx.shape
        dy = _f32c(dy)
        dx = torch.empty((B, C, H, W), dtype=F32, device=dy.device)
        call("itcv_avgpool2_bwd", ptr(dy), ptr(dx), B * C, H, W, stream())
        return dx


class Upsample2Fn(Function):
    @staticmethod
    def forward(ctx, x):
        x = _f32c(x)
        B, C, H, W = x.shape
        y = torch.empty((B, C, 2 * H, 2 * W), dtype=F32, device=x.device)
        call("itcv_upsample2_fwd", ptr(x), ptr(y), B * C, H, W, stream())
        ctx.shape = (B, C, H, W)
        return y

    @staticmethod
    @once_differentiable
    def backward(ctx, dy):
        B, C, H, W = ctx.shape
        dy = _f32c(dy)
        dx = torch.empty((B, C, H, W), dtype=F32, device=dy.device)
        call("itcv_upsample2_bwd", ptr(dy), ptr(dx), B * C, H, W, stream())
        return dx


class AddFn(Function):
    @staticmethod
    def forward(ctx, a, b):
        a, b = _f32c(a), _f32c(b)
        out = torch.empty_like(a)
        call("itcv_add", ptr(a), ptr(b), ptr(out), a.numel(), stream())
        return out

    @staticmethod
    def backward(ctx, g):
        return g, g


class ReparamFn(Function):

    @staticmethod
    def forward(ctx, mu, logvar, eps):
        mu, logvar, eps = _f32c(mu), _f32c(logvar), _f32c(eps)
        z = torch.empty_like(mu)
        call("itcv_reparam_fwd", ptr(mu), ptr(logvar), ptr(eps), ptr(z), mu.numel(), stream())
        ctx.save_for_backward(logvar, eps)
        return z

    @staticmethod
    @once_differentiable
    def backward(ctx, dz):
        logvar, eps = ctx.saved_tensors
        dz = _f32c(dz)
        dmu, dlv = torch.empty_like(dz), torch.empty_like(dz)
        call("itcv_reparam_bwd", ptr(dz), ptr(logvar), ptr(eps), ptr(dmu), ptr(dlv), dz.numel(), stream())
        return dmu, dlv, None


class KlRowsFn(Function):

    @staticmethod
    def forward(ctx, logvar, mu):
        logvar, mu = _f32c(logvar), _f32c(mu)
        B, D = logvar.shape
        kl = torch.empty((B,), dtype=F32, device=mu.device)
        call("itcv_kl_rows_fwd", ptr(logvar), ptr(mu), ptr(kl), B, D, stream())
        ctx.save_for_backward(logvar, mu)
        return kl

    @staticmethod
    @once_differentiable
    def backward(ctx, g):
        logvar, mu = ctx.saved_tensors
        B, D = logvar.shape
        g = _f32c(g)
        dlv, dmu = torch.empty_like(logvar), torch.empty_like(mu)
        call("itcv_kl_rows_bwd", ptr(g), ptr(logvar), ptr(mu), ptr(dlv), ptr(dmu), B, D, stream())
        return dlv, dmu


_REDUCTION = {"none": 0, "sum": 1, "mean": 2}


class KlLossFn(Function):

    @staticmethod
    def forward(ctx, logvar, mu, reduction, scale):
        logvar, mu = _f32c(logvar), _f32c(mu)
        B, D = logvar.shape
        out = torch.empty((B,) if reduction == 0 else (), dtype=F32, device=mu.device)
        call("itcv_kl_loss_fwd", ptr(logvar), ptr(mu), ptr(out), B, D, reduction, float(scale), stream())
        ctx.save_for_backward(logvar, mu)
        ctx.cfg = (B, D, reduction, float(scale))
        return out

    @staticmethod
    @once_differentiable
    def backward(ctx, g):
        logvar, mu = ctx.saved_tensors
        B, D, reduction, scale = ctx.cfg
        dlv, dmu = torch.empty_like(logvar), torch.empty_like(mu)
        call("itcv_kl_loss_bwd", ptr(_f32c(g)), ptr(logvar), ptr(mu), ptr(dlv), ptr(dmu), B, D, reduction, scale, stream())
        return dlv, dmu, None, None


class TcKlFn(Function):

    @staticmethod
    def forward(ctx, z, mu_all, logvar, dataset_size, row_offset, coef_tc, coef_kl, reduction):
        z, mu_all, logvar = _f32c(z), _f32c(mu_all), _f32c(logvar)
        Bl, D = z.shape
        Bt = mu_all.shape[0]
        dev = z.device
        out = torch.empty((Bl,) if reduction == 0 else (), dtype=F32, device=dev)
# ... 656 lines not shown
```

### intro-tc-vae_amd/solvers/intro.py

```python
from typing import Optional

import torch
from torch import Tensor

from hipvae import ddp
from hipvae.functional import ExpElboFn, SharedPass
from models import _has_hooks, bn_groups
from ops import noise, reparameterize
from solvers.vae import VAESolver


class IntroSolver(VAESolver):
    def __init__(self, dataset, model, batch_size: int, optimizer_e, optimizer_d, recon_loss_type: str,
                 beta_kl: float, beta_rec: float, beta_neg: float, gamma_r: float, device: torch.device,
                 use_amp: bool, grad_scaler, writer=None, test_iter: int = 1000, clip: Optional[float] = None):
        super().__init__(dataset, model, batch_size, optimizer_e, optimizer_d, recon_loss_type, beta_kl, beta_rec,
                         device, use_amp, grad_scaler, writer, test_iter, clip)
        self.beta_neg = beta_neg
        self.gamma_r = gamma_r
        self.batch_passes = True
        self.share_decoder_pass = True
        self._shared_pass = SharedPass()

    def _shares_pass(self) -> bool:
        return bool(self.batch_passes and self.share_decoder_pass) and not _has_hooks(self.model.decoder)

    def _schedule_key(self) -> tuple:
        return (bool(self.batch_passes), self._shares_pass())

    def _exp_elbo(self, rec_rows: Tensor, kl_rows: Tensor) -> Tensor:
        while rec_rows.dim() > 1:
            rec_rows = rec_rows.sum(-1)
        if rec_rows.is_cuda and rec_rows.shape == kl_rows.shape and rec_rows.dim() == 1:
            return ExpElboFn.apply(rec_rows, kl_rows, -2 * self.scale)
        return (-2 * self.scale * (rec_rows + kl_rows)).exp().mean()

    def _device_step(self, real: Tensor) -> Tensor:
        if not self.batch_passes:
            return self._device_step_unbatched(real)
        model, scale = self.model, self.scale
        cat = torch.cat

        def two():
            return bn_groups(2)

        share, shared = self._shares_pass(), self._shared_pass
        noise_batch = noise((real.size(0), model.zdim), self.device)
        self._set_trainable(encoder=True, decoder=False)
        real_mu, real_logvar = model.encode(real)
        z = reparameterize(real_mu, real_logvar)
        if share:
            self._set_trainable(encoder=True, decoder=True)
            with two(), shared.record():
                fake, rec = model.decoder(cat([noise_batch, z])).chunk(2)
            self._set_trainable(encoder=True, decoder=False)
        else:
            with two():
                fake, rec = model.decoder(cat([noise_batch, z])).chunk(2)
        loss_rec = self.compute_rec_loss(real, rec, reduction="mean")
        loss_e_real_kl = self.compute_kl_loss(z, real_mu, real_logvar, write=True)
        with two():
            mu2, logvar2 = model.encode(cat([rec.detach(), fake.detach()]))
        (rec_mu, fake_mu), (rec_logvar, fake_logvar) = mu2.chunk(2), logvar2.chunk(2)
        z_rec = reparameterize(rec_mu, rec_logvar)
        z_fake = reparameterize(fake_mu, fake_logvar)
        with two():
            rec_rec, rec_fake = model.decoder(cat([z_rec, z_fake])).chunk(2)
        kl_rec = self.compute_kl_loss(z_rec, rec_mu, rec_logvar, reduce="none", beta=self.beta_neg)
        kl_fake = self.compute_kl_loss(z_fake, fake_mu, fake_logvar, reduce="none", beta=self.beta_neg)
        expelbo_rec = self._exp_elbo(self.compute_rec_loss(rec, rec_rec, reduction="none"), kl_rec)
        expelbo_fake = self._exp_elbo(self.compute_rec_loss(fake, rec_fake, reduction="none"), kl_fake)
        loss_e = self._lincomb((scale, scale, 0.25, 0.25), loss_rec, loss_e_real_kl, expelbo_rec, expelbo_fake)
        shared.param_grads = False
        finish_average = self._backward(loss_e, ("encoder",), defer_average=True, retain_graph=share)
        shared.param_grads = True

        self._set_trainable(encoder=False, decoder=True)
        if share:
            loss_e, loss_e_real_kl, expelbo_fake = loss_e.detach(), loss_e_real_kl.detach(), expelbo_fake.detach()
            del (loss_rec, mu2, logvar2, rec_mu, fake_mu, rec_logvar, fake_logvar, z_rec, z_fake, rec_rec, rec_fake, kl_rec,
                 kl_fake, expelbo_rec, real_mu, real_logvar, z)
            shared.replay()
        else:
            with two():
                fake, rec = model.decoder(cat([noise_batch, z.detach()])).chunk(2)
        finish_average()
        norm_e = self._clip()
        self._step("encoder")
        loss_rec = self.compute_rec_loss(real, rec, reduction="mean", write=True)
        with two():
            mu2, logvar2 = model.encode(cat([rec, fake]))
        (rec_mu, fake_mu), (rec_logvar, fake_logvar) = mu2.chunk(2), logvar2.chunk(2)
        z_rec = reparameterize(rec_mu, rec_logvar)
        z_fake = reparameterize(fake_mu, fake_logvar)
        with two():
            rec_rec, rec_fake = model.decoder(cat([z_rec.detach(), z_fake.detach()])).chunk(2)
        g = self.gamma_r * self.beta_rec
        loss_rec_rec = self.compute_rec_loss(rec.detach(), rec_rec, reduction="mean", beta=g)
        loss_fake_rec = self.compute_rec_loss(fake.detach(), rec_fake, reduction="mean", beta=g)
        loss_d_rec_kl = self.compute_kl_loss(z_rec, rec_mu, rec_logvar)
        loss_d_fake_kl = self.compute_kl_loss(z_fake, fake_mu, fake_logvar)
        loss_d = self._lincomb((scale, 0.5 * scale, 0.5 * scale, 0.5 * scale, 0.5 * scale), loss_rec, loss_d_rec_kl,
                               loss_d_fake_kl, loss_rec_rec, loss_fake_rec)
        if share:
            shared.input_grad = False
            self._backward(loss_d, ("decoder",), inputs=self._params("decoder"))
        else:
            self._backward(loss_d, ("decoder",))
        norm_d = self._clip()
        self._step("decoder")

        stats = torch.stack([loss_e.detach(), loss_d.detach(), loss_e_real_kl.detach(), loss_rec.detach(),
                             expelbo_fake.detach(), loss_d_fake_kl.detach()])
        ddp.mean_scalars_(stats)
        zero = stats.new_zeros(1)
        self._last_fake = fake.detach() if self.writer else None
        return torch.cat([stats, norm_e if norm_e is not None else zero, norm_d if norm_d is not None else zero])

    def _device_step_unbatched(self, real: Tensor) -> Tensor:
        model, scale = self.model, self.scale
        noise_batch = noise((real.size(0), model.zdim), self.device)
        self._set_trainable(encoder=True, decoder=False)
        fake = model.sample(noise_batch)
        real_mu, real_logvar = model.encode(real)
        z = reparameterize(real_mu, real_logvar)
        rec = model.decoder(z)
        loss_rec = self.compute_rec_loss(real, rec, reduction="mean")
        loss_e_real_kl = self.compute_kl_loss(z, real_mu, real_logvar, write=True)
        rec_mu, rec_logvar, z_rec, rec_rec = model(rec.detach())
        fake_mu, fake_logvar, z_fake, rec_fake = model(fake.detach())
        kl_rec = self.compute_kl_loss(z_rec, rec_mu, rec_logvar, reduce="none", beta=self.beta_neg)
        kl_fake = self.compute_kl_loss(z_fake, fake_mu, fake_logvar, reduce="none", beta=self.beta_neg)
        expelbo_rec = self._exp_elbo(self.compute_rec_loss(rec, rec_rec, reduction="none"), kl_rec)
        expelbo_fake = self._exp_elbo(self.compute_rec_loss(fake, rec_fake, reduction="none"), kl_fake)
        loss_e = self._lincomb((scale, scale, 0.25, 0.25), loss_rec, loss_e_real_kl, expelbo_rec, expelbo_fake)
        finish_average = self._backward(loss_e, ("encoder",), defer_average=True)

        self._set_trainable(encoder=False, decoder=True)
        fake = model.sample(noise_batch)
        rec = model.decoder(z.detach())
        finish_average()
        norm_e = self._clip()
        self._step("encoder")
        loss_rec = self.compute_rec_loss(real, rec, reduction="mean", write=True)
        rec_mu, rec_logvar = model.encode(rec)
        z_rec = reparameterize(rec_mu, rec_logvar)
        fake_mu, fake_logvar = model.encode(fake)
        z_fake = reparameterize(fake_mu, fake_logvar)
        rec_rec = model.decode(z_rec.detach())
        rec_fake = model.decode(z_fake.detach())
        g = self.gamma_r * self.beta_rec
        loss_rec_rec = self.compute_rec_loss(rec.detach(), rec_rec, reduction="mean", beta=g)
        loss_fake_rec = self.compute_rec_loss(fake.detach(), rec_fake, reduction="mean", beta=g)
        loss_d_rec_kl = self.compute_kl_loss(z_rec, rec_mu, rec_logvar)
        loss_d_fake_kl = self.compute_kl_loss(z_fake, fake_mu, fake_logvar)
        loss_d = self._lincomb((scale, 0.5 * scale, 0.5 * scale, 0.5 * scale, 0.5 * scale), loss_rec, loss_d_rec_kl,
                               loss_d_fake_kl, loss_rec_rec, loss_fake_rec)
        self._backward(loss_d, ("decoder",))
# ... 31 lines not shown
```

### intro-tc-vae_amd/solvers/vae.py

```python
from typing import Optional

import torch
from torch import Tensor

from hipvae import ddp
from hipvae.functional import LinCombFn, conv_math_scope, deferred_wgrad_reduces, direct_grad_accumulation
from hipvae.flat import FlatGroup, clip_grad_norm, fused_update
from models import grad_free_parameters
from ops import kl_divergence, reconstruction_loss
from utils import SingletonWriter

try:
    from dataset import DisentanglementDataset
except Exception:
    class DisentanglementDataset:
        pass


class VAESolver:
    def __init__(self, dataset, model, batch_size: int, optimizer_e, optimizer_d, recon_loss_type: str,
                 beta_kl: float, beta_rec: float, device: torch.device, use_amp: bool, grad_scaler,
                 writer=None, test_iter: int = 1000, clip: Optional[float] = None):
        self.dataset = dataset
        if isinstance(dataset, DisentanglementDataset):
# ... 39 lines not shown
        self.write_scalar(SingletonWriter().cur_iter, "r_loss_unscaled", rec)
        return beta * rec

    @staticmethod
    def _lincomb(weights, *terms):
        if all(isinstance(t, Tensor) and t.numel() == 1 and t.is_cuda for t in terms):
            return LinCombFn.apply(tuple(weights), *terms)
        return sum(w * t for w, t in zip(weights, terms))

    def _params(self, part):
        mod = getattr(self.model, part)
        ent = self.__dict__.setdefault("_plists", {}).get(part)
        if ent is None or ent[0] is not mod:
            ent = self._plists[part] = (mod, list(mod.parameters()))
        return ent[1]

    def _group(self, part) -> FlatGroup:
        params = self._params(part)
        g = self._flat.get(part)
        if g is None or not g.owns(params):
            g = self._flat[part] = FlatGroup(params, inherit=g,
                                             grad_free=grad_free_parameters(getattr(self.model, part)))
        return g

    def _set_trainable(self, encoder: bool, decoder: bool):
        for p in self._params("encoder"):
            p.requires_grad = encoder
        for p in self._params("decoder"):
            p.requires_grad = decoder

    def _backward(self, loss, parts, defer_average=False, retain_graph=False, inputs=None):
        groups = [self._group(p) for p in parts]
        for g in groups:
            g.zero_grad()
        with direct_grad_accumulation(), deferred_wgrad_reduces():
            loss.backward(retain_graph=retain_graph, inputs=inputs)
        if defer_average:
            pending = [ddp.average_async(g.flat_g) for g in groups]
            return lambda: [f() for f in pending]
        for g in groups:
            ddp.average_(g.flat_g)
        return None

    def _clip(self):
        if not self.clip:
            return None
        return clip_grad_norm([self._group("encoder"), self._group("decoder")], self.clip)

    def _step(self, part):
        opt = self.optimizer_e if part == "encoder" else self.optimizer_d
        spec = fused_update(opt)
        if spec is None:
            opt.step()
        else:
            g = self._group(part)
            g.bind_optimizer(opt, spec)
            g.fused_step(spec)

    def enable_graph(self, flag: bool = True):
        self._graph_on = bool(flag)
        self._graph = None
        self._graphs, self._graph_warm = {}, {}
        return self

    def _graph_ok(self, specs=None):
        import ops
        if not (getattr(self, "_graph_on", False) and self.writer is None
                and (ddp.get() is None or ddp.graph_capturable())
                and ops._noise["queue"] is None and ops._noise["mode"] == "device"):
            return False
        if specs is None:
            specs = (fused_update(self.optimizer_e), fused_update(self.optimizer_d))
        return specs[0] is not None and specs[1] is not None

    def _run(self, real: Tensor) -> Tensor:
        with conv_math_scope(self.conv_math):
            return self._run_scoped(real)

    def _run_scoped(self, real: Tensor) -> Tensor:
        specs = (fused_update(self.optimizer_e), fused_update(self.optimizer_d)) if getattr(self, "_graph_on", False) \
            else None
        if not self._graph_ok(specs):
            return self._device_step(real)
        key = (tuple(real.shape), real.dtype, self.conv_math) + specs + self._schedule_key() \
            + (getattr(self, "kl_loss", None),)
        from hipvae.functional import bump_weight_epoch
        graphs = self.__dict__.setdefault("_graphs", {})
        ent = graphs.get(key)
        if ent is None:
            warm = self.__dict__.setdefault("_graph_warm", {})
            warm[key] = warm.get(key, 0) + 1
            if warm[key] <= (3 if not graphs else 1):
                return self._device_step(real)
            while len(graphs) >= 4:
                graphs.pop(next(iter(graphs)))
            ent = dict(inp=real.clone())
            bump_weight_epoch()
            torch.cuda.synchronize()
            ent["graph"] = torch.cuda.CUDAGraph()
            ddp.drain_pending_collectives()
            mode = "thread_local"
            with torch.cuda.graph(ent["graph"], capture_error_mode=mode):
                ent["out"] = self._device_step(ent["inp"])
            graphs[key] = ent
        self._graph, self._graph_key, self._graph_in, self._graph_out = ent["graph"], key, ent["inp"], ent["out"]
        ent["inp"].copy_(real)
        ent["graph"].replay()
        bump_weight_epoch()
        return ent["out"]

    def _schedule_key(self) -> tuple:
        return ()

    def _device_step(self, real: Tensor) -> Tensor:
        self._set_trainable(True, True)
        mu, logvar, z, rec = self.model(real)
        loss_rec = self.compute_rec_loss(real, rec, reduction="mean", write=True)
        loss_kl = self.compute_kl_loss(z, mu, logvar, write=True)
        loss = self._lincomb((self.scale, self.scale), loss_rec, loss_kl)
        self._backward(loss, ("decoder", "encoder"))
        norm = self._clip()
        self._step("encoder")
        self._step("decoder")
        stats = torch.stack([loss.detach(), loss_kl.detach(), loss_rec.detach()])
        ddp.mean_scalars_(stats)
        return torch.cat([stats, norm if norm is not None else stats.new_zeros(1)])

    def train_step(self, batch: Tensor, cur_iter: int) -> dict:
        if batch.dim() == 3:
            batch = batch.unsqueeze(0)
        real = batch.to(self.device)
        v_loss, v_kl, v_rec, v_norm = self._run(real).tolist()
        if v_loss != v_loss:
            raise RuntimeError
        if self.writer:
            self.write_scalars(cur_iter, losses=dict(r_loss=v_rec, kl_loss=v_kl))
            if self.clip:
                self.writer.add_scalar("total_norm", v_norm, global_step=cur_iter)
            self.write_gradient_norm(cur_iter)
            self._write_images_helper(real, cur_iter)
            self.write_disentanglemnt_scores(cur_iter)
            self.writer.flush()
        return {"loss_enc": v_loss, "loss_dec": v_loss, "loss_kl": v_kl, "loss_rec": v_rec,
                "L2": v_norm if self.clip else None}

    def _write_images_helper(self, batch, cur_iter):
        if self.writer is not None and cur_iter % self.test_iter == 0:
            noise = torch.randn(size=(batch.size(0), self.model.zdim), device=self.device)
            with torch.no_grad():
                fake = self.model.sample(noise)
            self.write_images(batch, fake, cur_iter)

    def write_images(self, batch, fake_batch, cur_iter):
        if self.writer is not None and cur_iter % self.test_iter == 0:
            with torch.no_grad():
                _, _, _, rec_det = self.model(batch, deterministic=True)
            k = min(batch.size(0), 16)
            grid = torch.cat([batch[:k], rec_det[:k], fake_batch[:k]], dim=0).data.cpu()
            self.writer.add_images("reconstructions", grid, global_step=cur_iter)

    def write_gradient_norm(self, cur_iter: int):
        grads = [p.grad.detach().norm(2) for p in self.model.encoder.fc.parameters() if p.grad is not None]
        if grads:
            self.writer.add_scalar("fc_grad_norm", torch.stack(grads).norm(2).item(), global_step=cur_iter)

    def write_scalar(self, cur_iter: int, tag: str, value: Tensor):
        if self.writer and value.dim() == 0:
            self.writer.add_scalar(tag, value.data.item(), global_step=cur_iter)

    def write_scalars(self, cur_iter: int, losses: dict, **kwargs):
        if self.writer is not None:
            self.write_losses(cur_iter, losses)
            for name, value in kwargs.items():
                self.writer.add_scalar(name, value, global_step=cur_iter)

    def write_losses(self, cur_iter: int, losses: dict):
        if self.writer is not None:
            self.writer.add_scalars("losses", losses, global_step=cur_iter)

    def write_disentanglemnt_scores(self, cur_iter: int, num_samples: int = 10000):
        if self.writer is None or not isinstance(self.dataset, DisentanglementDataset) or cur_iter % self.test_iter:
            return
        extras = tuple(self.extra_scores or ())
        unknown = [e for e in extras if e not in ("factor_vae", "sap")]
        if unknown:
            raise ValueError(f"extra_scores: unknown score(s) {unknown} (known: 'factor_vae', 'sap')")
        with_dci = isinstance(self.device_scores, str) and self.device_scores == "all+dci"
        M = None
        if not with_dci:
            try:
                from evaluation import metrics as M
            except Exception:
                M = None
        native = (M is None) if self.device_scores is None else bool(self.device_scores)
# ... 46 lines not shown
```

Before: 4126 images/s.

## Skip backward work for the dead batch half in the shared encoder pass

During the encoder backward of the shared decoder pass, only one of the two batched groups (rec vs fake) carries gradient to the encoder. The change marks that group as live and threads a live image range through the conv dgrad, BN backward, activation, upsample and sigmoid backward paths. Dead groups get zero gradients and zeroed BN sums instead of computed ones. This roughly halves the input-gradient work in that pass, at the cost of new sub-batch conv entry points, extra graph-key state, and fallbacks (blocking) for ops that cannot honour the range.

```diff
diff --git a/include/itcv_hip.h b/include/itcv_hip.h
--- a/include/itcv_hip.h
+++ b/include/itcv_hip.h
@@ -49,6 +49,9 @@
 int itcv_conv2d_fwd_bf16p_st(const void* xplanes, const void* wp, const float* bias, float* y, int B, int Ci, int H,
                              int W, int Co, int KS, int up2, int ns, float* tile_stats, void* ws, size_t ws_bytes,
                              void* stream);
+int itcv_conv2d_fwd_bf16p_sub(const void* xplanes, const void* wp, const float* bias, float* y, int B, int Ci, int H,
+                              int W, int Co, int KS, int up2, int ns, int b0, int nb, void* ws, size_t ws_bytes,
+                              void* stream);
 int itcv_conv2d_wgrad_bf16p_supported(int B, int Ci, int H, int W, int Co, int KS);
 size_t itcv_conv2d_wgrad_bf16p_workspace(int B, int Ci, int H, int W, int Co, int KS);
 int itcv_conv2d_wgrad_bf16p(const void* xplanes, const void* dyplanes, float* dw, int B, int Ci, int H, int W,
@@ -145,6 +148,11 @@
                       const float* beta, const float* skip, double* dsums, float* dx, float* dskip, void* dx_planes,
                       int ns, float* dgamma, float* dbeta, int accumulate, int B, int C, int H, int W, float slope,
                       int pool, int up2, void* ws, size_t ws_bytes, size_t plane_stride, int groups, void* stream);
+int itcv_bn_train_bwd_live(const float* x, const float* dy, const float* mean, const float* rstd, const float* gamma,
+                           const float* beta, const float* skip, double* dsums, float* dx, float* dskip, void* dx_planes,
+                           int ns, float* dgamma, float* dbeta, int accumulate, int B, int C, int H, int W, float slope,
+                           int pool, int up2, void* ws, size_t ws_bytes, size_t plane_stride, int groups, int live0,
+                           int nlive, void* stream);
 
 #define ITCV_BN_PATH_ONE_BLOCK 0
 #define ITCV_BN_PATH_SLICED_FOLD 1
diff --git a/intro-tc-vae_amd/csrc/conv_igemm.hip b/intro-tc-vae_amd/csrc/conv_igemm.hip
--- a/intro-tc-vae_amd/csrc/conv_igemm.hip
+++ b/intro-tc-vae_amd/csrc/conv_igemm.hip
@@ -2411,26 +2411,36 @@
   return plan_fwd_planes(B, Ci, H, W, Co, KS, ns, true).stat_tiles;
 }
 
-int itcv_conv2d_fwd_bf16p_st(const void* xplanes, const void* wp, const float* bias, float* y, int B, int Ci, int H,
-                             int W, int Co, int KS, int up2, int fmt, float* tile_stats, void* ws, size_t ws_bytes,
-                             void* stream) {
+static int fwd_planes_run(const void* xplanes, const void* wp, const float* bias, float* y, int B, int Ci, int H, int W,
+                          int Co, int KS, int up2, int fmt, float* tile_stats, void* ws, size_t ws_bytes, int b0, int nb,
+                          void* stream) {
   if (int e = check_dims("itcv_conv2d_fwd_bf16p", B, Ci, H, W, Co, KS)) return e;
   ITCV_REQUIRE(xplanes && wp && y && fmt_ok(fmt), "itcv_conv2d_fwd_bf16p");
+  ITCV_REQUIRE(b0 >= 0 && nb >= 1 && b0 + nb <= B && (nb == B || !tile_stats), "itcv_conv2d_fwd_bf16p(image range)");
   const int f16 = fmt == ITCV_PLANES_F16X2, ns = planes_of_fmt(fmt);
   if (tile_stats && (f16 || !itcv_conv2d_fwd_bf16p_stat_tiles(B, Ci, H, W, Co, KS, ns)))
     return fail("%s: tile statistics are not available for this shape / format (see itcv_conv2d_fwd_bf16p_stat_tiles)",
                 "itcv_conv2d_fwd_bf16p_st");
-  const size_t in_plane = (size_t)B * (Ci / 8) * (up2 ? (H / 2) * (W / 2) : H * W);
+  const size_t in_image = (size_t)(Ci / 8) * (up2 ? (H / 2) * (W / 2) : H * W), in_plane = (size_t)B * in_image;
   const u32x4* xp = static_cast<const u32x4*>(xplanes);
   const ScaleRec* xrec = f16 ? reinterpret_cast<const ScaleRec*>(xp + 2 * in_plane) : nullptr;
+  xp += (size_t)b0 * in_image;
+  y += (size_t)b0 * Co * H * W;
   if (!itcv_conv2d_bf16s_supported(Ci, Co, KS))
     return fail("%s: shape not supported by the split-bf16 kernel (Ci %% 32, Co > 32, KS 1/3)", "itcv_conv2d_fwd_bf16p");
   if (up2) ITCV_REQUIRE(H % 2 == 0 && W % 2 == 0, "itcv_conv2d_fwd_bf16p(up2)");
-  const size_t out_elems = (size_t)B * Co * H * W;
-  const FwdPlanP p = plan_fwd_planes(B, Ci, H, W, Co, KS, ns, tile_stats != nullptr);
+  const size_t out_elems = (size_t)nb * Co * H * W;
+  FwdPlanP p = plan_fwd_planes(B, Ci, H, W, Co, KS, ns, tile_stats != nullptr);
   if (int e = check_ws("itcv_conv2d_fwd_bf16p", ws, ws_bytes, p.ws_need)) return e;
+  if (nb != B) {
+    p.nt = (int)(((long long)nb * H * W + p.bn - 1) / p.bn);
+    if (p.path == FwdPath::Band || p.path == FwdPath::BandPersistent) {
+      const int ids = cdiv(p.nt, 8) * 8 * p.mt, pb = g_opt.band_persist_blocks;
+      p.path = (pb > 0 && ids > pb) ? FwdPath::BandPersistent : FwdPath::Band;
+    }
+  }
   const bool split = p.splits > 1;
-  const double flop = 2.0 * B * H * W * (double)Co * Ci * KS * KS;
+  const double flop = 2.0 * nb * H * W * (double)Co * Ci * KS * KS;
   hipStream_t st = S(stream);
   if (p.path != FwdPath::Planes128) {
     ConvArgsP2 a;
@@ -2438,9 +2448,9 @@
     a.wp = static_cast<const u32x4*>(wp);
     a.bias = split ? nullptr : bias;
     a.y = split ? static_cast<float*>(ws) : y;
-    a.B = B, a.Ci = Ci, a.H = H, a.Co = Co;
+    a.B = nb, a.Ci = Ci, a.H = H, a.Co = Co;
     a.Mp = p.mt * p.bm;
-    a.N = B * H * W;
+    a.N = nb * H * W;
     a.mt = p.mt, a.nt = p.nt, a.cpt = p.cpt, a.cpt_per_split = p.cps;
     a.SR = p.SR, a.NSEG = p.NSEG, a.NP = p.NP, a.NPC = p.NPC, a.PXB = p.PXB;
     a.h_shift = log2_exact(H);
@@ -2462,9 +2472,9 @@
     a.wp = static_cast<const u32x4*>(wp);
     a.bias = split ? nullptr : bias;
     a.y = split ? static_cast<float*>(ws) : y;
-    a.B = B, a.Ci = Ci, a.H = H, a.W = W, a.Co = Co;
+    a.B = nb, a.Ci = Ci, a.H = H, a.W = W, a.Co = Co;
     a.Mp = p.mt * p.bm;
-    a.N = B * H * W;
+    a.N = nb * H * W;
     a.mt = p.mt, a.nt = p.nt, a.ktiles = p.ktiles, a.ktiles_per_split = p.kps;
     a.slab_stride = split ? out_elems : 0;
     a.plane_stride = in_plane;
@@ -2479,6 +2489,18 @@
     ITCV_CHECK_LAUNCH("itcv_conv2d_fwd_bf16p");
   }
   return reduce_fwd_splits("itcv_conv2d_fwd_bf16p(reduce)", ws, bias, y, out_elems, p.splits, H * W, Co, st);
+}
+
+int itcv_conv2d_fwd_bf16p_st(const void* xplanes, const void* wp, const float* bias, float* y, int B, int Ci, int H,
+                             int W, int Co, int KS, int up2, int fmt, float* tile_stats, void* ws, size_t ws_bytes,
+                             void* stream) {
+  return fwd_planes_run(xplanes, wp, bias, y, B, Ci, H, W, Co, KS, up2, fmt, tile_stats, ws, ws_bytes, 0, B, stream);
+}
+
+int itcv_conv2d_fwd_bf16p_sub(const void* xplanes, const void* wp, const float* bias, float* y, int B, int Ci, int H,
+                              int W, int Co, int KS, int up2, int fmt, int b0, int nb, void* ws, size_t ws_bytes,
+                              void* stream) {
+  return fwd_planes_run(xplanes, wp, bias, y, B, Ci, H, W, Co, KS, up2, fmt, nullptr, ws, ws_bytes, b0, nb, stream);
 }
 
 size_t itcv_conv2d_wgrad_workspace(int B, int Ci, int H, int W, int Co, int KS) {
diff --git a/intro-tc-vae_amd/csrc/norm_act.hip b/intro-tc-vae_amd/csrc/norm_act.hip
--- a/intro-tc-vae_amd/csrc/norm_act.hip
+++ b/intro-tc-vae_amd/csrc/norm_act.hip
@@ -17,7 +17,11 @@
   size_t ps;
   int cs;
   int G;
+  int lv0, lvn;
 };
+__device__ __forceinline__ bool bn_dead(const BnGrp& g, uint32_t group) {
+  return g.lvn > 0 && (group < (uint32_t)g.lv0 || group >= (uint32_t)(g.lv0 + g.lvn));
+}
 
 struct BnFinal {
   double count;
@@ -531,8 +535,10 @@
   const float mu = mean[c], rs = rstd[c];
   double s1 = 0.0, s2 = 0.0;
   float gmax = 0.f, xmax = 0.f;
+  const bool dead = bn_dead(grp, FUSED ? (uint32_t)gi : gz);
+  const uint32_t gend = (dead && !MX) ? beg : end;
   constexpr int U = 4;
-  for (uint32_t i0 = beg + threadIdx.x * 4; i0 < end; i0 += kRedThreads * 4 * U) {
+  for (uint32_t i0 = beg + threadIdx.x * 4; i0 < gend; i0 += kRedThreads * 4 * U) {
     float4 xv4[U], g4[U], k4[U];
     bool ok[U];
 #pragma unroll
@@ -544,9 +550,9 @@
       const uint32_t h = fdiv(hw, W, w_shift), w = hw - h * W;
       const uint32_t bc = b * C + c;
       xv4[u] = *reinterpret_cast<const float4*>(x + (size_t)bc * HW + hw);
-      g4[u] = upstream4<MODE>(dy, bc, h, w, H, W);
-    }
-    if (skip) {
+      g4[u] = dead ? make_float4(0.f, 0.f, 0.f, 0.f) : upstream4<MODE>(dy, bc, h, w, H, W);
+    }
+    if (skip && !dead) {
 #pragma unroll
       for (int u = 0; u < U; ++u) {
         const uint32_t iu = i0 + (uint32_t)u * kRedThreads * 4, i = iu < end ? iu : i0;
@@ -692,7 +698,7 @@
       rec->scale = pscale, rec->inv = 1.f / pscale, rec->pad[0] = rec->pad[1] = 0.f;
     }
   }
-  const uint32_t zg = gridDim.z - 1 - blockIdx.z;
+  const uint32_t zg = (uint32_t)grp.lv0 + gridDim.z - 1 - blockIdx.z;
   {
     const size_t g = zg;
     x += g * grp.xs, dy += g * grp.dys, planes += g * grp.ps, mean += g * grp.cs, rstd += g * grp.cs;
@@ -722,10 +728,13 @@
         s_m1[threadIdx.x] = (float)(s1 / count), s_m2[threadIdx.x] = (float)(s2 / count);
         if (g < C8 && g * per_plane >= base) {
           sm.dsums_out[(size_t)gz * 2 * C + c] = s1, sm.dsums_out[(size_t)gz * 2 * C + C + c] = s2;
-          if (gz == 0) {
+          if (gz == (uint32_t)grp.lv0) {
+            for (uint32_t gg = 0; gg < G; ++gg)
+              if (bn_dead(grp, gg)) sm.dsums_out[(size_t)gg * 2 * C + c] = 0.0, sm.dsums_out[(size_t)gg * 2 * C + C + c] = 0.0;
             float db = (sm.accumulate && sm.dbeta) ? sm.dbeta[c] : 0.f, dg = (sm.accumulate && sm.dgamma) ? sm.dgamma[c] : 0.f;
             db += (float)s1, dg += (float)s2;
-            for (uint32_t gg = 1; gg < G; ++gg) {
+            for (uint32_t gg = 0; gg < G; ++gg) {
+              if (gg == gz) continue;
               const double* pg = sm.part + (size_t)gg * sm.splits * 2 * C;
               db += (float)fold_strided(0.0, pg + c, (size_t)2 * C, sm.splits);
               dg += (float)fold_strided(0.0, pg + C + c, (size_t)2 * C, sm.splits);
@@ -1265,34 +1274,44 @@
   return 0;
 }
 
-int itcv_bn_train_bwd(const float* x, const float* dy, const float* mean, const float* rstd, const float* gamma,
-                      const float* beta, const float* skip, double* dsums, float* dx, float* dskip, void* dx_planes,
-                      int ns, float* dgamma, float* dbeta, int accumulate, int B, int C, int H, int W, float slope,
-                      int pool, int up2, void* ws, size_t ws_bytes, size_t plane_stride, int groups, void* stream) {
+int itcv_bn_train_bwd_live(const float* x, const float* dy, const float* mean, const float* rstd, const float* gamma,
+                           const float* beta, const float* skip, double* dsums, float* dx, float* dskip, void* dx_planes,
+                           int ns, float* dgamma, float* dbeta, int accumulate, int B, int C, int H, int W, float slope,
+                           int pool, int up2, void* ws, size_t ws_bytes, size_t plane_stride, int groups, int live0,
+                           int nlive, void* stream) {
   ITCV_REQUIRE(x && dy && mean && rstd && gamma && beta && dsums && (dx || dx_planes) && B > 0 && C > 0,
                "itcv_bn_train_bwd");
   ITCV_REQUIRE(!(pool && up2), "itcv_bn_train_bwd(pool and up2 are exclusive)");
-  const double bn_el = (double)(groups > 1 ? groups : 1) * B * C * H * W;
+  const int ngroups = groups > 1 ? groups : 1;
+  ITCV_REQUIRE(live0 >= 0 && nlive >= 1 && live0 + nlive <= ngroups, "itcv_bn_train_bwd_live(live range inside the groups)");
+  const bool all_live = nlive == ngroups;
+  const double bn_el = (double)nlive * B * C * H * W;
   ProfScope bn_prof(S(stream), kProfBnBwd, ilog2_exact(W) >= 0 ? ilog2_exact(W) : 0, C / 8, pool ? 1 : (up2 ? 2 : 0), dx_planes ? ns : 0,
                     bn_el * 4.0 * (1.0 + (pool ? 0.25 : (up2 ? 4.0 : 1.0)) + (skip ? 1.0 : 0.0)) +
                         bn_el * ((dx_planes ? 4.0 : 0.0) + (dx ? 4.0 : 0.0) + (dskip ? 4.0 : 0.0)));
   if (groups > 1) ITCV_REQUIRE(!dx_planes || plane_stride, "itcv_bn_train_bwd(groups need the plane stride of the whole tensor)");
-  const BnPlan p = bn_plan(true, B, C, H, W, pool, up2, groups, dx_planes != nullptr, ns, plane_stride, ws ? ws_bytes : 0,
-                           false);
+  BnPlan p = bn_plan(true, B, C, H, W, pool, up2, groups, dx_planes != nullptr, ns, plane_stride, ws ? ws_bytes : 0, false);
+  if (!all_live) p.grp.lv0 = live0, p.grp.lvn = nlive, p.agrid.z = nlive;
   const size_t ws_need = p.ws_need;
   if (p.f16 && groups > 1 && (p.path == BnPath::PerGroup || !(ws && ws_bytes >= ws_need)))
     return fail("%s: fp16 gradient planes need the merged group path (W %% 4 == 0, planes, a workspace of itcv_bn_workspace * groups)",
                 "itcv_bn_train_bwd");
   if (p.path == BnPath::PerGroup) {
     const BnGrp& s = p.grp;
-    for (int g = 0; g < groups; ++g)
+    for (int g = 0; g < groups; ++g) {
+      if (g < live0 || g >= live0 + nlive) {
+        if (hipMemsetAsync(dsums + (size_t)g * 2 * C, 0, (size_t)2 * C * sizeof(double), S(stream)) != hipSuccess)
+          return fail("%s: clearing a dead group's sums failed", "itcv_bn_train_bwd_live");
+        continue;
+      }
       if (int e = itcv_bn_train_bwd(x + g * s.xs, dy + g * s.dys, mean + (size_t)g * C, rstd + (size_t)g * C, gamma, beta,
                                     skip ? skip + g * s.xs : nullptr, dsums + (size_t)g * 2 * C, dx ? dx + g * s.xs : nullptr,
                                     dskip ? dskip + g * s.xs : nullptr,
                                     dx_planes ? static_cast<u32x4*>(dx_planes) + g * s.ps : nullptr, ns, dgamma, dbeta,
-                                    (accumulate || g > 0) ? 1 : 0, B, C, H, W, slope, pool, up2, ws, ws_bytes, plane_stride,
-                                    1, stream))
+                                    (accumulate || g > live0) ? 1 : 0, B, C, H, W, slope, pool, up2, ws, ws_bytes,
+                                    plane_stride, 1, stream))
         return e;
+    }
     return 0;
   }
   if (p.f16) ITCV_REQUIRE(ws && ws_bytes >= ws_need, "itcv_bn_train_bwd(workspace, fp16 planes)");
@@ -1307,6 +1326,15 @@
                              H, W, slope, fold, mx, S(stream));
 }
 
+int itcv_bn_train_bwd(const float* x, const float* dy, const float* mean, const float* rstd, const float* gamma,
+                      const float* beta, const float* skip, double* dsums, float* dx, float* dskip, void* dx_planes,
+                      int ns, float* dgamma, float* dbeta, int accumulate, int B, int C, int H, int W, float slope,
+                      int pool, int up2, void* ws, size_t ws_bytes, size_t plane_stride, int groups, void* stream) {
+  return itcv_bn_train_bwd_live(x, dy, mean, rstd, gamma, beta, skip, dsums, dx, dskip, dx_planes, ns, dgamma, dbeta,
+                                accumulate, B, C, H, W, slope, pool, up2, ws, ws_bytes, plane_stride, groups, 0,
+                                groups > 1 ? groups : 1, stream);
+}
+
 static_assert((int)BnPath::OneBlock == ITCV_BN_PATH_ONE_BLOCK && (int)BnPath::SlicedFold == ITCV_BN_PATH_SLICED_FOLD &&
                   (int)BnPath::SlicedCombine == ITCV_BN_PATH_SLICED_COMBINE && (int)BnPath::Fallback == ITCV_BN_PATH_FALLBACK &&
                   (int)BnPath::PerGroup == ITCV_BN_PATH_PER_GROUP && (int)BnPath::TileStats == ITCV_BN_PATH_TILE_STATS,
diff --git a/intro-tc-vae_amd/hipvae/abi.py b/intro-tc-vae_amd/hipvae/abi.py
--- a/intro-tc-vae_amd/hipvae/abi.py
+++ b/intro-tc-vae_amd/hipvae/abi.py
@@ -42,6 +42,7 @@
     "itcv_conv2d_fwd_bf16p": (i32, [p, p, p, p] + [i32] * 8 + [p, sz, p]),
     "itcv_conv2d_fwd_bf16p_stat_tiles": (i32, [i32] * 7),
     "itcv_conv2d_fwd_bf16p_st": (i32, [p, p, p, p] + [i32] * 8 + [p, p, sz, p]),
+    "itcv_conv2d_fwd_bf16p_sub": (i32, [p, p, p, p] + [i32] * 10 + [p, sz, p]),
     "itcv_conv2d_wgrad_bf16p_supported": (i32, [i32] * 6),
     "itcv_conv2d_wgrad_bf16p_workspace": (sz, [i32] * 6),
     "itcv_conv2d_wgrad_bf16p": (i32, [p, p, p] + [i32] * 9 + [p, sz, p]),
@@ -95,6 +96,8 @@
     "itcv_bn_replay_max_descs": (i32, []),
     "itcv_bn_train_bwd": (i32, [p, p, p, p, p, p, p, p, p, p, p, i32, p, p, i32, i32, i32, i32, i32, f32, i32, i32, p,
                                 sz, sz, i32, p]),
+    "itcv_bn_train_bwd_live": (i32, [p, p, p, p, p, p, p, p, p, p, p, i32, p, p, i32, i32, i32, i32, i32, f32, i32, i32, p,
+                                     sz, sz, i32, i32, i32, p]),
     "itcv_bn_plan_query": (i32, [i32] * 10 + [sz, i32, p, p]),
     "itcv_lrelu_fwd": (i32, [p, p, sz, f32, p]),
     "itcv_lrelu_bwd": (i32, [p, p, p, sz, f32, p]),
diff --git a/intro-tc-vae_amd/hipvae/functional.py b/intro-tc-vae_amd/hipvae/functional.py
--- a/intro-tc-vae_amd/hipvae/functional.py
+++ b/intro-tc-vae_amd/hipvae/functional.py
@@ -65,6 +65,8 @@
     def __init__(self):
         self.param_grads = True
         self.input_grad = True
+        self.live = None
+        self.live_blockers = []
         self.records = []
         self._first = False
         self._pool = {}
@@ -75,6 +77,7 @@
         prev, _SHARED_PASS[0] = _SHARED_PASS[0], self
         self.records, self._first = [], True
         self.param_grads = self.input_grad = True
+        self.live, self.live_blockers = None, []
         try:
             yield self
         finally:
@@ -98,6 +101,38 @@
 def _shared_ok(ctx, what):
     sp = ctx.shared
     return sp is None or getattr(sp, what)
+
+
+def _block_live(why):
+    sp = _SHARED_PASS[0]
+    if sp is not None and why not in sp.live_blockers:
+        sp.live_blockers.append(why)
+
+
+def _live_images(ctx, B):
+    sp = getattr(ctx, "shared", None)
+    if sp is None or sp.live is None or sp.param_grads or sp.live_blockers:
+        return None
+    g, G = sp.live
+    if B % G:
+        raise abi.HipExtensionError(f"SharedPass.live: batch {B} is not {G} equal groups")
+    return g * (B // G), B // G
+
+
+def _new_grad(like_or_shape, device=None, live=None):
+    t = torch.empty_like(like_or_shape) if device is None else torch.empty(like_or_shape, dtype=F32, device=device)
+    if live is not None and _POISON[0]:
+        t.fill_(float("nan"))
+    return t
+
+
+def _dgrad_sub_kind(Co, Ci, KS):
+    ns = _planes_ns(Co, Ci, KS, False)
+    if ns:
+        return None if (_two(ns) and lib.itcv_conv2d_small_cout_bf16p_supported(Co, Ci, KS)) else "planes"
+    if lib.itcv_conv2d_small_cout_supported(Ci, KS):
+        return None
+    return "small" if lib.itcv_conv2d_small_cin_supported(Co, KS) else None
 
 
 def replay_bn_running(records, tables=None):
@@ -285,7 +320,9 @@
 _SCIN_MFMA = [True]
 
 
-def conv_apply(x, weight, w4, for_dgrad, bias, B, Ci, H, W, Co, KS, up2):
+def conv_apply(x, weight, w4, for_dgrad, bias, B, Ci, H, W, Co, KS, up2, out=None):
+    if out is not None and (up2 or lib.itcv_conv2d_small_cout_supported(Co, KS) or not lib.itcv_conv2d_small_cin_supported(Ci, KS)):
+        raise abi.HipExtensionError("conv_apply: an output tensor is taken by the small-cin kernels only")
     if not up2 and lib.itcv_conv2d_small_cout_supported(Co, KS):
         y = torch.empty((B, Co, H, W), dtype=F32, device=x.device)
 
@@ -293,7 +330,7 @@
              stream())
         return y
     if not up2 and lib.itcv_conv2d_small_cin_supported(Ci, KS):
-        y = torch.empty((B, Co, H, W), dtype=F32, device=x.device)
+        y = out if out is not None else torch.empty((B, Co, H, W), dtype=F32, device=x.device)
         fmt = _NS[_CONV_MATH[0]]
         if _SCIN_MFMA[0] and _two(fmt) and lib.itcv_conv2d_small_cin_bf16x3_supported(Ci, Co, KS, W):
             amax = absmax_parts(x) if (fmt == F16X2 and for_dgrad) else None
@@ -339,7 +376,15 @@
 _FUSE_STATS = [False]
 
 
-def conv_apply_planes(xp, weight, w4, for_dgrad, bias, B, Ci, H, W, Co, KS, up2, ns, want_stats=False):
+def conv_apply_planes(xp, weight, w4, for_dgrad, bias, B, Ci, H, W, Co, KS, up2, ns, want_stats=False, live=None):
+    if live is not None:
+        wp = packed_weight(weight, w4, for_dgrad, ns)
+        y = _new_grad((B, Co, H, W), xp.device, live)
+        nws = lib.itcv_conv2d_fwd_bf16p_workspace(B, Ci, H, W, Co, KS, ns)
+        ws = _ws(nws, xp.device) if nws else None
+        call("itcv_conv2d_fwd_bf16p_sub", ptr(xp), ptr(wp), ptr(bias), ptr(y), B, Ci, H, W, Co, KS, int(up2), ns, live[0],
+             live[1], ptr(ws), nws, stream())
+        return y
     if not up2 and _two(ns) and lib.itcv_conv2d_small_cout_bf16p_supported(Ci, Co, KS):
         y = torch.empty((B, Co, H, W), dtype=F32, device=xp.device)
         call("itcv_conv2d_small_cout_fwd_bf16p", ptr(xp), ptr(w4), ptr(bias), ptr(y), B, Ci, H, W, Co, KS, int(for_dgrad),
@@ -650,6 +695,8 @@
         ctx.cfg = (B, Ci, H, W, Co, KS, up2, bias is not None, (Hs, Ws))
         ctx.shared = _SHARED_PASS[0]
         ctx.shared_first = ctx.shared is not None and ctx.shared._claim_first()
+        if ctx.shared is not None and _dgrad_sub_kind(Co, Ci, KS) is None:
+            _block_live(f"conv {Ci}->{Co} k{KS}: data gradient without a sub-range form in mode {_CONV_MATH[0]}")
         return y
 
     @staticmethod
@@ -666,16 +713,29 @@
         wg_planes = need_w and _wgrad_planes_ok(B, Ci, H, W, Co, KS)
         dyp = None
         fmt2 = F16X2 if _NS[_CONV_MATH[0]] == F16X2 else 2
+        live = _live_images(ctx, B) if need_x else None
+        if live is not None and _dgrad_sub_kind(Co, Ci, KS) is None:
+            raise abi.HipExtensionError("Conv2dFn.backward: conv math mode changed inside a shared pass")
+        if live is not None and ns_d and _tagged_planes(dy, ns_d) is None:
+            full = torch.zeros_like(dy)
+            full[live[0]:live[0] + live[1]] = dy[live[0]:live[0] + live[1]]
+            dy = full
         if ns_d or wg_planes:
             dyp = planes_of(dy, ns_d if ns_d else fmt2, gradient=True)
         if need_x:
             if ns_d:
-                dx = conv_apply_planes(dyp, weight, weight, 1, None, B, Co, H, W, Ci, KS, False, ns_d)
+                dx = conv_apply_planes(dyp, weight, weight, 1, None, B, Co, H, W, Ci, KS, False, ns_d, live=live)
+            elif live is not None:
+                r = slice(live[0], live[0] + live[1])
+                dx = _new_grad((B, Ci, H, W), dy.device, live)
+                conv_apply(_require_fp32(dy, "Conv2dFn.backward")[r], weight, weight, 1, None, live[1], Co, H, W, Ci, KS, False,
+                           out=dx[r])
             else:
                 dx = conv_apply(_require_fp32(dy, "Conv2dFn.backward"), weight, weight, 1, None, B, Co, H, W, Ci, KS, False)
             if up2:
-                lo = torch.empty((B, Ci, H // 2, W // 2), dtype=F32, device=dy.device)
-                call("itcv_upsample2_bwd", ptr(dx), ptr(lo), B * Ci, H // 2, W // 2, stream())
+                lo = _new_grad((B, Ci, H // 2, W // 2), dy.device, live)
+                b0, nb = live if live is not None else (0, B)
+                call("itcv_upsample2_bwd", ptr(dx[b0:b0 + nb]), ptr(lo[b0:b0 + nb]), nb * Ci, H // 2, W // 2, stream())
                 dx = lo
         wg5 = _wgrad5_mode(Ci, H, W, Co, KS, up2) if need_w else None
         if wg5 == "predict" and xp is None and x is None:
@@ -774,6 +834,9 @@
         dev = x.device
         shared = _SHARED_PASS[0]
         uvar = None
+        if shared is not None and (not training or _world(group) != 1 or skip is not None or G != int(bn_groups)
+                                   or not lib.itcv_bn_act_planes_supported(C, H, W, 0)):
+            _block_live(f"BatchNorm C={C} {H}x{W}: eval / Sync-BN / skip input / a shape the planes kernels do not take")
         if shared is not None and training:
             mean, uvar = shared._stats(G, C, dev)
         else:
@@ -862,7 +925,10 @@
             dgamma = torch.empty_like(gamma) if need_g else None
             dbeta = torch.empty_like(beta) if need_b else None
             pg, pb = dgamma, dbeta
-        dx = torch.empty_like(x)
+        live = _live_images(ctx, B) if world == 1 else None
+        if live is not None and (ctx.shared.live[1] != G or skip is not None):
+            raise abi.HipExtensionError("BnActFn.backward: SharedPass.live does not match the BatchNorm groups of the pass")
+        dx = _new_grad(x, live=live)
         dskip = torch.empty_like(x) if (skip is not None and ctx.needs_input_grad[3]) else None
         dxp, pstride = None, 0
         if grad_planes:
@@ -872,9 +938,13 @@
         if world == 1:
             ws = _ws(nws, dev)
             local = torch.empty((G, 2 * C), dtype=torch.float64, device=dev)
-            call("itcv_bn_train_bwd", ptr(x), ptr(dy), ptr(mean), ptr(rstd), ptr(gamma), ptr(beta), ptr(skip), ptr(local),
-                 ptr(dx) if write_dx else None, ptr(dskip), ptr(dxp), grad_planes, ptr(pg), ptr(pb), 1 if direct else 0, Bg,
-                 C, H, W, slope, pool, 0, ptr(ws), nws, pstride, G, stream())
+            head = (ptr(x), ptr(dy), ptr(mean), ptr(rstd), ptr(gamma), ptr(beta), ptr(skip), ptr(local),
+                    ptr(dx) if write_dx else None, ptr(dskip), ptr(dxp), grad_planes, ptr(pg), ptr(pb), 1 if direct else 0, Bg,
+                    C, H, W, slope, pool, 0, ptr(ws), nws, pstride, G)
+            if live is None:
+                call("itcv_bn_train_bwd", *head, stream())
+            else:
+                call("itcv_bn_train_bwd_live", *head, ctx.shared.live[0], 1, stream())
         for g in (range(G) if world != 1 else ()):
             r = slice(g * Bg, (g + 1) * Bg)
             acc = 1 if (direct or g > 0) else 0
@@ -907,6 +977,7 @@
         call("itcv_lrelu_fwd", ptr(x), ptr(y), x.numel(), float(slope), stream())
         ctx.save_for_backward(x)
         ctx.slope = float(slope)
+        ctx.shared = _SHARED_PASS[0]
         return y
 
     @staticmethod
@@ -914,6 +985,12 @@
     def backward(ctx, dy):
         (x,) = ctx.saved_tensors
         dy = _f32c(dy)
+        live = _live_images(ctx, x.shape[0]) if x.dim() else None
+        if live is not None:
+            r = slice(live[0], live[0] + live[1])
+            dx = torch.zeros_like(x)
+            call("itcv_lrelu_bwd", ptr(x[r]), ptr(dy[r]), ptr(dx[r]), x[r].numel(), ctx.slope, stream())
+            return dx, None
         dx = torch.empty_like(x)
         call("itcv_lrelu_bwd", ptr(x), ptr(dy), ptr(dx), x.numel(), ctx.slope, stream())
         return dx, None
@@ -926,6 +1003,7 @@
         y = torch.empty_like(x)
         call("itcv_sigmoid_fwd", ptr(x), ptr(y), x.numel(), stream())
         ctx.save_for_backward(y)
+        ctx.shared = _SHARED_PASS[0]
         return y
 
     @staticmethod
@@ -933,8 +1011,10 @@
     def backward(ctx, dy):
         (y,) = ctx.saved_tensors
         dy = _f32c(dy)
-        dx = torch.empty_like(y)
-        call("itcv_sigmoid_bwd", ptr(y), ptr(dy), ptr(dx), y.numel(), stream())
+        live = _live_images(ctx, y.shape[0]) if y.dim() else None
+        dx = _new_grad(y, live=live)
+        r = slice(None) if live is None else slice(live[0], live[0] + live[1])
+        call("itcv_sigmoid_bwd", ptr(y[r]), ptr(dy[r]), ptr(dx[r]), y[r].numel(), stream())
         return dx
 
 
@@ -945,6 +1025,7 @@
         B, C, H, W = x.shape
         y = torch.empty((B, C, H // 2, W // 2), dtype=F32, device=x.device)
         call("itcv_avgpool2_fwd", ptr(x), ptr(y), B * C, H, W, stream())
+        _block_live("average pool")
         ctx.shape = (B, C, H, W)
         return y
 
@@ -966,6 +1047,7 @@
         y = torch.empty((B, C, 2 * H, 2 * W), dtype=F32, device=x.device)
         call("itcv_upsample2_fwd", ptr(x), ptr(y), B * C, H, W, stream())
         ctx.shape = (B, C, H, W)
+        ctx.shared = _SHARED_PASS[0]
         return y
 
     @staticmethod
@@ -973,8 +1055,10 @@
     def backward(ctx, dy):
         B, C, H, W = ctx.shape
         dy = _f32c(dy)
-        dx = torch.empty((B, C, H, W), dtype=F32, device=dy.device)
-        call("itcv_upsample2_bwd", ptr(dy), ptr(dx), B * C, H, W, stream())
+        live = _live_images(ctx, B)
+        b0, nb = live if live is not None else (0, B)
+        dx = _new_grad((B, C, H, W), dy.device, live)
+        call("itcv_upsample2_bwd", ptr(dy[b0:b0 + nb]), ptr(dx[b0:b0 + nb]), nb * C, H, W, stream())
         return dx
 
 
@@ -984,6 +1068,7 @@
         a, b = _f32c(a), _f32c(b)
         out = torch.empty_like(a)
         call("itcv_add", ptr(a), ptr(b), ptr(out), a.numel(), stream())
+        _block_live("residual add")
         return out
 
     @staticmethod
diff --git a/intro-tc-vae_amd/solvers/intro.py b/intro-tc-vae_amd/solvers/intro.py
--- a/intro-tc-vae_amd/solvers/intro.py
+++ b/intro-tc-vae_amd/solvers/intro.py
@@ -20,6 +20,7 @@
         self.gamma_r = gamma_r
         self.batch_passes = True
         self.share_decoder_pass = True
+        self.skip_dead_half = True
         self._shared_pass = SharedPass()
 
     def _shares_pass(self) -> bool:
@@ -27,6 +28,9 @@
 
     def _schedule_key(self) -> tuple:
         return (bool(self.batch_passes), self._shares_pass())
+
+    def _graph_key_extra(self) -> tuple:
+        return (bool(self.skip_dead_half),)
 
     def _exp_elbo(self, rec_rows: Tensor, kl_rows: Tensor) -> Tensor:
         while rec_rows.dim() > 1:
@@ -72,8 +76,9 @@
         expelbo_fake = self._exp_elbo(self.compute_rec_loss(fake, rec_fake, reduction="none"), kl_fake)
         loss_e = self._lincomb((scale, scale, 0.25, 0.25), loss_rec, loss_e_real_kl, expelbo_rec, expelbo_fake)
         shared.param_grads = False
+        shared.live = (1, 2) if (share and self.skip_dead_half and ddp.get() is None) else None
         finish_average = self._backward(loss_e, ("encoder",), defer_average=True, retain_graph=share)
-        shared.param_grads = True
+        shared.param_grads, shared.live = True, None
 
         self._set_trainable(encoder=False, decoder=True)
         if share:
diff --git a/intro-tc-vae_amd/solvers/vae.py b/intro-tc-vae_amd/solvers/vae.py
--- a/intro-tc-vae_amd/solvers/vae.py
+++ b/intro-tc-vae_amd/solvers/vae.py
@@ -145,7 +145,7 @@
             else None
         if not self._graph_ok(specs):
             return self._device_step(real)
-        key = (tuple(real.shape), real.dtype, self.conv_math) + specs + self._schedule_key() \
+        key = (tuple(real.shape), real.dtype, self.conv_math) + specs + self._graph_key_extra() + self._schedule_key() \
             + (getattr(self, "kl_loss", None),)
         from hipvae.functional import bump_weight_epoch
         graphs = self.__dict__.setdefault("_graphs", {})
@@ -173,6 +173,9 @@
         return ent["out"]
 
     def _schedule_key(self) -> tuple:
+        return ()
+
+    def _graph_key_extra(self) -> tuple:
         return ()
 
     def _device_step(self, real: Tensor) -> Tensor:
```

Result: faster. 4173 images/s, median of 6 (+1.1%).
